# acgtun/hsearch

Measured on AMD Instinct MI355X. Metric: motif queries/sec (LSH probe + verify, index resident in HBM), higher is better.
Workload: dtype f64

## Files before the change

### hsearch_amd/capi.py

```python
import ctypes as C
import os

import numpy as np

_HERE = os.path.dirname(os.path.abspath(__file__))

HS_OK, HS_ERR_INVALID, HS_ERR_NO_DEVICE, HS_ERR_HIP, HS_ERR_CAPACITY, HS_ERR_STATE, \
    HS_ERR_KEY_COLLISION, HS_ERR_NOMEM, HS_ERR_IO, HS_ERR_PEER = range(10)
_STATUS = ["HS_OK", "HS_ERR_INVALID", "HS_ERR_NO_DEVICE", "HS_ERR_HIP", "HS_ERR_CAPACITY",
           "HS_ERR_STATE", "HS_ERR_KEY_COLLISION", "HS_ERR_NOMEM", "HS_ERR_IO", "HS_ERR_PEER"]

_ALPHABET = "ARNDCQEGHILKMFPSTWYV"

EXPORTS = ["hs_create", "hs_destroy", "hs_last_error", "hs_get_profile", "hs_get_params", "hs_version",
           "hs_set_verify_mode", "hs_set_hash_mode", "hs_set_option", "hs_set_bucket_partition", "hs_set_multiprobe", "hs_probe_buckets", "hs_wait_event", "hs_set_planes", "hs_self_join", "hs_self_join_range", "hs_clustering",
           "hs_clustering_begin", "hs_clustering_table_edges", "hs_clustering_table_apply",
           "hs_clustering_end",
           "hs_embed_codes", "hs_hash_codes", "hs_hash_points", "hs_key_string", "hs_key_fingerprint",
           "hs_key_strings_equal", "hs_index_build", "hs_index_build_subset", "hs_index_build_windows", "hs_index_shard_begin", "hs_index_shard_hash_dev", "hs_index_shard_group_dev",
           "hs_index_shard_tuples_dev", "hs_index_shard_finish_dev", "hs_index_shard_end", "hs_index_save", "hs_index_load", "hs_index_file_check", "hs_klsh_draw_planes", "hs_klsh_codes",
           "hs_index_info_get", "hs_query", "hs_query_dev", "hs_query_codes", "hs_query_codes_dev", "hs_bruteforce",
           "hs_bruteforce_topk", "hs_merge_first_table_dev", "hs_query_radii", "hs_query_radii_dev",
           "hs_bruteforce_radii", "hs_annotate", "hs_annotate_dev", "hs_merge_best", "hs_components", "hs_components_dev",
           "hs_components_range", "hs_components_range_dev", "hs_components_merge", "hs_degrees", "hs_degrees_dev",
           "hs_degrees_range", "hs_degrees_range_dev", "hs_dbscan", "hs_dbscan_dev", "hs_dbscan_edges",
           "hs_cluster_profile", "hs_cluster_profile_dev", "hs_cluster_radii", "hs_cluster_radii_dev",
           "hs_cluster_summary_codes", "hs_msf", "hs_msf_dev", "hs_msf_edges", "hs_msf_cut", "hs_core_distance",
           "hs_core_distance_dev", "hs_density_tree", "hs_density_tree_dev", "hs_density_tree_edges",
           "hs_density_tree_cut", "hs_query_topk", "hs_query_topk_dev", "hs_self_knn", "hs_self_knn_range",
           "hs_self_knn_dev", "hs_self_knn_range_dev", "hs_topk_merge", "hs_seq_match", "hs_seq_match_dev",
           "hs_window_id_start", "hs_seq_match_hits", "hs_seq_match_merge", "hs_join6_tables", "hs_join6_thresholds",
           "hs_join6_selftest", "hs_index_append", "hs_index_append_dev", "hs_index_append_windows",
           "hs_index_table_append"]

TOPK_MAX = 64
NO_ID = 0xffffffff
NOISE = 0xffffffff


class HsError(RuntimeError):
    def __init__(self, status, message):
        self.status = status
        name = _STATUS[status] if 0 <= status < len(_STATUS) else str(status)
        super().__init__("%s: %s" % (name, message))


class _Params(C.Structure):
    _fields_ = [("k", C.c_uint32), ("K", C.c_uint32), ("L", C.c_uint32), ("W", C.c_double),
                ("device", C.c_int32), ("alphabet", C.c_uint32)]


class _Profile(C.Structure):
    _fields_ = [("ms_hash", C.c_double), ("ms_sort", C.c_double), ("ms_gather", C.c_double),
                ("ms_probe", C.c_double), ("ms_verify", C.c_double), ("ms_finalize", C.c_double),
                ("ms_total", C.c_double), ("candidates", C.c_uint64), ("provisional", C.c_uint64),
                ("hits", C.c_uint64), ("verify_launches", C.c_uint64), ("join_batches", C.c_uint64),
                ("ms_join", C.c_double), ("join_items", C.c_uint64), ("join_pairs", C.c_uint64),
                ("join_pairs_issued", C.c_uint64), ("join_i8_batches", C.c_uint64),
                ("hash_values", C.c_uint64), ("hash_flagged", C.c_uint64),
                ("join_row_bytes", C.c_uint32), ("join_wide", C.c_uint32), ("join_items_resident", C.c_uint64),
                ("join_async_retries", C.c_uint64), ("queries_recognised", C.c_uint64),
                ("join_f6_batches", C.c_uint64), ("append_rebuilds", C.c_uint64),
                ("append_new_buckets", C.c_uint64)]


class _IndexInfo(C.Structure):
    _fields_ = [("n", C.c_uint64), ("device_bytes", C.c_uint64), ("n_buckets", C.c_uint64 * 32),
                ("max_bucket", C.c_uint64 * 32), ("key_seed", C.c_uint32)]


class _DbscanCounts(C.Structure):
    _fields_ = [("n_clusters", C.c_uint64), ("n_core", C.c_uint64), ("n_border", C.c_uint64),
                ("n_noise", C.c_uint64), ("n_edges", C.c_uint64)]


class _MsfInfo(C.Structure):
    _fields_ = [("n_tree_edges", C.c_uint64), ("n_components", C.c_uint64), ("n_graph_edges", C.c_uint64),
                ("rounds", C.c_uint32), ("resident", C.c_uint32)]


class _DensityInfo(C.Structure):
    _fields_ = [("n_tree_edges", C.c_uint64), ("n_clusters", C.c_uint64), ("n_core", C.c_uint64),
                ("n_graph_edges", C.c_uint64), ("rounds", C.c_uint32), ("resident", C.c_uint32),
                ("self_joins", C.c_uint32)]


profile_fields = [f[0] for f in _Profile._fields_]

_libs = {}


def lib_path(hooks=False):
    if hooks:
        return os.path.join(_HERE, "libhsearch_amd_hooks.so")
    return os.environ.get("HSEARCH_AMD_LIB") or os.path.join(_HERE, "libhsearch_amd.so")


def load(hooks=False):
    if hooks not in _libs:
        try:
            import torch
        except Exception:
            pass
        path = lib_path(hooks)
        if not os.path.exists(path):
            raise ImportError("%s is missing: run `python -c 'import __graft_entry__ as g; "
                              "g.build()'` (or make -C hsearch_amd/csrc)" % path)
        lib = C.CDLL(path)
        lib.hs_version.restype = C.c_char_p
        lib.hs_last_error.restype = C.c_char_p
        lib.hs_last_error.argtypes = [C.c_void_p]
        lib.hs_destroy.restype = None
        lib.hs_destroy.argtypes = [C.c_void_p]
        lib.hs_key_string.restype = C.c_uint32
        lib.hs_key_fingerprint.restype = C.c_uint64
        lib.hs_key_strings_equal.restype = C.c_int
        if hasattr(lib, "hs_query_radii"):
            for fn in (lib.hs_query_radii, lib.hs_query_radii_dev):
                fn.restype = C.c_int
                fn.argtypes = [C.c_void_p, C.c_void_p, C.c_void_p, C.c_uint64, C.c_void_p, C.c_void_p, C.c_void_p,
                               C.c_void_p, C.c_void_p, C.c_uint64, C.POINTER(C.c_uint64), C.c_void_p]
            lib.hs_bruteforce_radii.restype = C.c_int
            lib.hs_bruteforce_radii.argtypes = [C.c_void_p, C.c_void_p, C.c_uint64, C.c_void_p, C.c_void_p,
                                                C.c_void_p, C.c_void_p, C.c_uint64, C.POINTER(C.c_uint64)]
        if hasattr(lib, "hs_annotate"):
            for fn in (lib.hs_annotate, lib.hs_annotate_dev):
                fn.restype = C.c_int
                fn.argtypes = [C.c_void_p, C.c_void_p, C.c_void_p, C.c_uint64, C.c_double, C.c_void_p, C.c_void_p,
                               C.c_void_p, C.c_void_p, C.c_void_p, C.c_uint64, C.POINTER(C.c_uint64)]
            lib.hs_merge_best.restype = C.c_int
            lib.hs_merge_best.argtypes = [C.c_void_p, C.c_void_p, C.c_void_p, C.c_void_p, C.c_uint64, C.c_void_p,
                                          C.c_void_p, C.c_void_p, C.c_void_p, C.c_uint64, C.POINTER(C.c_uint64)]
        if hasattr(lib, "hs_components"):
            for fn in (lib.hs_components, lib.hs_components_dev):
                fn.restype = C.c_int
                fn.argtypes = [C.c_void_p, C.c_double, C.c_int, C.c_void_p, C.POINTER(C.c_uint64),
                               C.POINTER(C.c_uint64)]
            for fn in (lib.hs_components_range, lib.hs_components_range_dev):
                fn.restype = C.c_int
                fn.argtypes = [C.c_void_p, C.c_uint64, C.c_uint64, C.c_double, C.c_int, C.c_void_p,
                               C.POINTER(C.c_uint64), C.POINTER(C.c_uint64)]
            lib.hs_components_merge.restype = C.c_int
            lib.hs_components_merge.argtypes = [C.c_void_p, C.c_uint64, C.c_uint64, C.c_void_p, C.POINTER(C.c_uint64)]
        if hasattr(lib, "hs_dbscan"):
            for fn in (lib.hs_degrees, lib.hs_degrees_dev):
                fn.restype = C.c_int
                fn.argtypes = [C.c_void_p, C.c_double, C.c_int, C.c_void_p, C.POINTER(C.c_uint64)]
            for fn in (lib.hs_degrees_range, lib.hs_degrees_range_dev):
                fn.restype = C.c_int
                fn.argtypes = [C.c_void_p, C.c_uint64, C.c_uint64, C.c_double, C.c_int, C.c_void_p,
                               C.POINTER(C.c_uint64)]
            for fn in (lib.hs_dbscan, lib.hs_dbscan_dev):
                fn.restype = C.c_int
                fn.argtypes = [C.c_void_p, C.c_double, C.c_int, C.c_uint32, C.c_void_p, C.c_void_p,
                               C.POINTER(_DbscanCounts)]
            lib.hs_dbscan_edges.restype = C.c_int
            lib.hs_dbscan_edges.argtypes = [C.c_void_p, C.c_void_p, C.c_uint64, C.c_uint64, C.c_uint32, C.c_void_p,
                                            C.c_void_p, C.POINTER(_DbscanCounts)]
        if hasattr(lib, "hs_cluster_profile"):
            for fn in (lib.hs_cluster_profile, lib.hs_cluster_profile_dev):
                fn.restype = C.c_int
                fn.argtypes = [C.c_void_p, C.c_void_p, C.c_uint32, C.c_void_p, C.c_void_p, C.c_void_p, C.c_void_p,
                               C.c_uint64, C.POINTER(C.c_uint64)]
            for fn in (lib.hs_cluster_radii, lib.hs_cluster_radii_dev):
                fn.restype = C.c_int
                fn.argtypes = [C.c_void_p, C.c_void_p, C.c_uint32, C.c_void_p, C.c_uint64, C.c_void_p, C.c_void_p,
                               C.c_void_p]
            lib.hs_cluster_summary_codes.restype = C.c_int
            lib.hs_cluster_summary_codes.argtypes = [C.c_void_p, C.c_uint64, C.c_uint32, C.c_void_p, C.c_uint32,
                                                     C.c_void_p, C.c_uint32, C.c_void_p, C.c_uint64, C.c_void_p,
                                                     C.c_void_p, C.c_void_p, C.c_void_p, C.c_void_p, C.c_void_p,
                                                     C.c_void_p, C.c_uint64, C.POINTER(C.c_uint64)]
        if hasattr(lib, "hs_msf"):
            for fn in (lib.hs_msf, lib.hs_msf_dev):
                fn.restype = C.c_int
                fn.argtypes = [C.c_void_p, C.c_double, C.c_int, C.c_void_p, C.c_void_p, C.c_void_p, C.c_uint64,
                               C.c_void_p, C.POINTER(_MsfInfo)]
            lib.hs_msf_edges.restype = C.c_int
            lib.hs_msf_edges.argtypes = [C.c_void_p, C.c_void_p, C.c_void_p, C.c_uint64, C.c_uint64, C.c_void_p,
                                         C.c_void_p, C.c_void_p, C.c_uint64, C.c_void_p, C.POINTER(_MsfInfo)]
            lib.hs_msf_cut.restype = C.c_int
            lib.hs_msf_cut.argtypes = [C.c_void_p, C.c_void_p, C.c_void_p, C.c_uint64, C.c_uint64, C.c_double,
                                       C.c_void_p, C.POINTER(C.c_uint64)]
        if hasattr(lib, "hs_density_tree"):
            for fn in (lib.hs_core_distance, lib.hs_core_distance_dev):
# ... 279 lines not shown
    assert ei.ndim == 1 and ei.shape == ej.shape == dist.shape
    n = int(n)
    room = n if cap is None else int(cap)
    lo = np.empty(room, dtype=np.uint32)
    hi = np.empty(room, dtype=np.uint32)
    od = np.empty(room, dtype=np.float64)
    label = np.empty(n, dtype=np.uint32) if want_label else None
    info = _MsfInfo()
    st = load().hs_msf_edges(_vp(ei), _vp(ej), _vp(dist), len(ei), n, _vp(lo), _vp(hi), _vp(od), room,
                             _vp(label) if want_label else None, C.byref(info))
    if st != HS_OK:
        e = HsError(st, "hs_msf_edges")
        e.needed = int(info.n_tree_edges)
        raise e
    return _msf_dict(info, lo, hi, od, label)


def msf_cut(tree, r, n=None, out=None):
    lo = np.ascontiguousarray(tree["lo"], dtype=np.uint32)
    hi = np.ascontiguousarray(tree["hi"], dtype=np.uint32)
    dist = np.ascontiguousarray(tree["dist"], dtype=np.float64)
    assert lo.ndim == 1 and lo.shape == hi.shape == dist.shape
    n = len(tree["label"]) if n is None else int(n)
    if out is None:
        out = np.empty(n, dtype=np.uint32)
    assert out.dtype == np.uint32 and out.shape == (n,) and out.flags["C_CONTIGUOUS"]
    nc = C.c_uint64(0)
    st = load().hs_msf_cut(_vp(lo), _vp(hi), _vp(dist), len(lo), n, float(r), _vp(out), C.byref(nc))
    if st != HS_OK:
        raise HsError(st, "hs_msf_cut")
    return dict(label=out, n_components=int(nc.value))


def _density_dict(info, lo, hi, w, label, core):
    m = int(info.n_tree_edges)
    res = dict(lo=lo[:m], hi=hi[:m], w=w[:m], **{f[0]: int(getattr(info, f[0])) for f in _DensityInfo._fields_})
    if label is not None:
        res["label"] = label
    if core is not None:
        res["core"] = core
    return res


def density_tree_edges(ei, ej, dist, n, min_pts, want_label=True, cap=None):
    ei = np.ascontiguousarray(ei, dtype=np.uint32)
    ej = np.ascontiguousarray(ej, dtype=np.uint32)
    dist = np.ascontiguousarray(dist, dtype=np.float64)
    assert ei.ndim == 1 and ei.shape == ej.shape == dist.shape
    n = int(n)
    room = n if cap is None else int(cap)
    lo = np.empty(room, dtype=np.uint32)
    hi = np.empty(room, dtype=np.uint32)
    w = np.empty(room, dtype=np.float64)
    label = np.empty(n, dtype=np.uint32) if want_label else None
    core = np.empty(n, dtype=np.float64)
    info = _DensityInfo()
    st = load().hs_density_tree_edges(_vp(ei), _vp(ej), _vp(dist), len(ei), n, int(min_pts), _vp(lo), _vp(hi), _vp(w),
                                      room, _vp(label) if want_label else None, _vp(core), C.byref(info))
    if st != HS_OK:
        e = HsError(st, "hs_density_tree_edges")
        e.needed = int(info.n_tree_edges)
        raise e
    return _density_dict(info, lo, hi, w, label, core)


def density_tree_cut(tree, r, n=None, out=None):
    lo = np.ascontiguousarray(tree["lo"], dtype=np.uint32)
    hi = np.ascontiguousarray(tree["hi"], dtype=np.uint32)
    w = np.ascontiguousarray(tree["w"], dtype=np.float64)
    core = np.ascontiguousarray(tree["core"], dtype=np.float64)
    assert lo.ndim == 1 and lo.shape == hi.shape == w.shape and core.ndim == 1
    n = len(core) if n is None else int(n)
    assert len(core) == n
    if out is None:
        out = np.empty(n, dtype=np.uint32)
    assert out.dtype == np.uint32 and out.shape == (n,) and out.flags["C_CONTIGUOUS"]
    nc = C.c_uint64(0)
    st = load().hs_density_tree_cut(_vp(lo), _vp(hi), _vp(w), len(lo), _vp(core), n, float(r), _vp(out), C.byref(nc))
    if st != HS_OK:
        raise HsError(st, "hs_density_tree_cut")
    return dict(label=out, n_clusters=int(nc.value))


def cluster_summary_codes(codes, label, min_size=1, coords=None, centers=None, want_counts=False, want_radii=True,
                          cap=None):
    codes = np.ascontiguousarray(codes, dtype=np.uint8)
    label = np.ascontiguousarray(label, dtype=np.uint32)
    assert codes.ndim == 2 and label.shape == (codes.shape[0],)
    n, k = codes.shape
    alpha = 20
    if coords is not None:
        coords = np.ascontiguousarray(coords, dtype=np.float64)
        assert coords.ndim == 2 and coords.shape[1] == 8
        alpha = coords.shape[0]
    room = n // max(1, int(min_size)) if cap is None else int(cap)
    if centers is not None:
        centers = np.ascontiguousarray(centers, dtype=np.float64)
        assert centers.ndim == 2 and centers.shape[1] == 8 * k
    ol = np.empty(room, dtype=np.uint32)
    osz = np.empty(room, dtype=np.uint32)
    cen = np.empty((room, 8 * k), dtype=np.float64)
    cnt = np.empty((room, k, alpha), dtype=np.uint32) if want_counts else None
    mx = np.empty(room, dtype=np.float64) if want_radii else None
    rad = np.empty(room, dtype=np.float64) if want_radii else None
    med = np.empty(room, dtype=np.uint32) if want_radii else None
    n_out = C.c_uint64(0)
    opt = lambda a: None if a is None else _vp(a)
    st = load().hs_cluster_summary_codes(_vp(codes), n, k, opt(coords), alpha if coords is not None else 0, _vp(label),
                                         int(min_size), opt(centers), 0 if centers is None else centers.shape[0],
                                         _vp(ol), _vp(osz), opt(cnt), _vp(cen), opt(mx), opt(rad), opt(med), room,
                                         C.byref(n_out))
    if st != HS_OK:
        e = HsError(st, "hs_cluster_summary_codes")
        e.needed = int(n_out.value)
        raise e
    m = int(n_out.value)
    res = dict(label=ol[:m], size=osz[:m], centroid=cen[:m])
    if want_counts:
        res["counts"] = cnt[:m]
    if want_radii:
        res.update(max_d2=mx[:m], radius=rad[:m], medoid=med[:m])
    return res


def join6_tables(coords):
    coords = np.ascontiguousarray(coords, dtype=np.float64)
    A = coords.shape[0]
    s = C.c_double(0.0)
    codes = np.zeros((32, 4), dtype=np.uint8)
    e, r = np.zeros(32), np.zeros(32)
    pair = np.zeros((1024, 2), dtype=np.uint32)
    lib = load()
    st = lib.hs_join6_tables(_vp(coords), C.c_uint32(A), C.byref(s), _vp(codes), _vp(e), _vp(r), _vp(pair))
    if st:
        raise HsError(st, "hs_join6_tables")
    return dict(s=s.value, codes=codes[:A], e=e[:A], r=r[:A], pair=pair)


def join6_thresholds(coords, kmers, r2):
    coords = np.ascontiguousarray(coords, dtype=np.float64)
    kmers = np.ascontiguousarray(kmers, dtype=np.uint8)
    n, k = kmers.shape
    r2 = np.ascontiguousarray(np.broadcast_to(np.asarray(r2, dtype=np.float64), (n,)))
    rho64, c64 = np.zeros(n, dtype=np.int64), np.zeros(n, dtype=np.int64)
    rho0 = C.c_int64(0)
    rec = np.zeros((n, 4), dtype=np.uint32)
    st = load().hs_join6_thresholds(_vp(coords), C.c_uint32(coords.shape[0]), _vp(kmers), C.c_uint64(n), C.c_uint32(k),
                                    _vp(r2), _vp(rho64), _vp(c64), C.byref(rho0), _vp(rec))
    if st:
        raise HsError(st, "hs_join6_thresholds")
    return dict(rho64=rho64, c64=c64, rho0_64=rho0.value, rec=rec)


def join6_selftest(device=0, variant=0):
    n = C.c_uint64(0)
    bad = (C.c_uint32 * 4)()
    st = load().hs_join6_selftest(C.c_int(device), C.c_int(variant), C.byref(n), bad)
    if st:
        raise HsError(st, "hs_join6_selftest")
    return int(n.value), tuple(int(x) for x in bad)


def index_file_check(path):
    err = C.create_string_buffer(512)
    st = load().hs_index_file_check(str(path).encode(), err, C.c_uint32(len(err)))
    if st != HS_OK:
        raise HsError(st, err.value.decode())


def index_table_append(ids, dir_key, dir_start, dir_tuple, block_ints, seed=0, out=None):
    ids = np.ascontiguousarray(ids, dtype=np.uint32)
    dir_key = np.ascontiguousarray(dir_key, dtype=np.uint64)
    dir_start = np.ascontiguousarray(dir_start, dtype=np.uint32)
    dir_tuple = np.ascontiguousarray(dir_tuple, dtype=np.int32)
    block_ints = np.ascontiguousarray(block_ints, dtype=np.int32)
    n, nb, m = len(ids), len(dir_key), block_ints.shape[0]
    K = block_ints.shape[1] if block_ints.ndim == 2 else dir_tuple.shape[1]
    assert len(dir_start) == nb + 1 and dir_tuple.size == nb * K and block_ints.size == m * K
    lib = load()
    nb_out, collided = C.c_uint64(0), C.c_uint32(0)

    def call(o_ids, o_key, o_start, o_tuple, cap):
        return lib.hs_index_table_append(_vp(ids), _vp(dir_key), _vp(dir_start), _vp(dir_tuple), C.c_uint64(n),
                                         C.c_uint64(nb), _vp(block_ints), C.c_uint64(m), C.c_uint32(K), C.c_uint32(seed),
                                         o_ids, o_key, o_start, o_tuple, C.c_uint64(cap), C.byref(nb_out),
                                         C.byref(collided))
    if out is None:
        st = call(None, None, None, None, 0)
        if st == HS_OK and collided.value:
            return None
        if st not in (HS_OK, HS_ERR_CAPACITY):
            raise HsError(st, "hs_index_table_append")
        cap = int(nb_out.value)
        out = (np.empty(n + m, dtype=np.uint32), np.empty(cap, dtype=np.uint64), np.empty(cap + 1, dtype=np.uint32),
               np.empty((cap, K), dtype=np.int32))
    o_ids, o_key, o_start, o_tuple = out
    assert len(o_ids) >= n + m and len(o_start) >= len(o_key) + 1 and o_tuple.size >= len(o_key) * K
    st = call(_vp(o_ids), _vp(o_key), _vp(o_start), _vp(o_tuple), len(o_key))
    if st != HS_OK:
        raise HsError(st, "hs_index_table_append")
    if collided.value:
        return None
    nbo = int(nb_out.value)
    return o_ids[:n + m], o_key[:nbo], o_start[:nbo + 1], o_tuple.reshape(-1, K)[:nbo]


KLSH_NONE = 0xffffffffffffffff
_REDUCED_CLASS = {c: k for k, grp in enumerate(["AST", "RKEDQ", "NH", "C", "G", "IVLM", "FYW", "P"])
                  for c in grp}


def klsh_draw_planes(feat=512, bits=16, sigma=0.2):
    w = np.empty((bits, feat)); b = np.empty(bits); t = np.empty(bits)
    st = load().hs_klsh_draw_planes(C.c_uint32(feat), C.c_uint32(bits), C.c_double(sigma), _vp(w),
                                    _vp(b), _vp(t))
    if st != HS_OK:
        raise HsError(st, "hs_klsh_draw_planes")
    return w, b, t


def klsh_codes(classes, seq_start, w, b, t, device=0):
    classes = np.ascontiguousarray(classes, dtype=np.uint8)
    seq_start = np.ascontiguousarray(seq_start, dtype=np.uint64)
    w = np.ascontiguousarray(w, dtype=np.float64); b = np.ascontiguousarray(b, dtype=np.float64)
    t = np.ascontiguousarray(t, dtype=np.float64)
    n_seq = len(seq_start) - 1
    codes = np.empty(n_seq, dtype=np.uint64); unc = np.empty(n_seq, dtype=np.uint64)
    err = C.create_string_buffer(256)
    st = load().hs_klsh_codes(C.c_int(device), _vp(classes), C.c_uint64(len(classes)), _vp(seq_start),
                              C.c_uint64(n_seq), _vp(w), _vp(b), _vp(t), C.c_uint32(w.shape[0]),
                              _vp(codes), _vp(unc), err, C.c_uint32(256))
    if st != HS_OK:
        raise HsError(st, err.value.decode())
    return codes, unc


class Engine:

    def __init__(self, k, K, L, W, a, b, device=0, coords=None, hooks=False, options=None):
        self._lib = load(hooks)
        self.k, self.K, self.L, self.W = int(k), int(K), int(L), float(W)
        self.d = 8 * self.k
        self.T = 0
        a = np.ascontiguousarray(a, dtype=np.float64)
        b = np.ascontiguousarray(b, dtype=np.float64)
        assert a.shape == (self.L, self.K, self.d), a.shape
        assert b.shape == (self.L, self.K), b.shape
        cptr = None
        if coords is not None:
            coords = np.ascontiguousarray(coords, dtype=np.float64)
            assert coords.ndim == 2 and coords.shape[1] == 8 and 1 <= coords.shape[0] <= 32
            cptr = _vp(coords)
        params = _Params(self.k, self.K, self.L, self.W, int(device),
                         0 if coords is None else coords.shape[0])
        self._h = C.c_void_p()
        st = self._lib.hs_create(C.byref(params), _vp(a), _vp(b), cptr, C.byref(self._h))
        if st != HS_OK:
            msg = self._lib.hs_last_error(self._h).decode() if self._h else ""
            if self._h:
                self._lib.hs_destroy(self._h)
                self._h = C.c_void_p()
            raise HsError(st, msg or "hs_create failed (is a gfx950 GPU visible?)")
        for name, value in (options or {}).items():
            self.set_option(name, value)

    def _check(self, st):
        if st != HS_OK:
            raise HsError(st, self._lib.hs_last_error(self._h).decode())

    def set_verify_mode(self, mode):
        self._check(self._lib.hs_set_verify_mode(self._h, {"auto": 0, "stream": 1, "join": 2, "join16": 3}[mode]))

    def set_hash_mode(self, mode, eps_scale=1.0):
        self._check(self._lib.hs_set_hash_mode(self._h, {"auto": 0, "exact": 1, "mfma": 2}[mode],
                                               C.c_double(eps_scale)))

    OPTIONS = {"query_batch": 1, "seg_mode": 2, "join_resident": 3, "recognise_kmers": 4, "build_grouping": 5,
               "wide_rows": 6, "refine8": 7, "self_codes": 8, "sort_hits": 10, "sync_items": 11,
               "join_min_q": 12, "join_min_m": 13, "sort_from_bit": 14, "build_serial": 15,
               "join_xcd_run": 16, "probe_records": 17, "join_chunk": 18, "summary_chunk": 19, "summary_rows": 20,
               "msf_edge_budget": 21, "join_f6": 22}

    def set_option(self, name, value):
        self._check(self._lib.hs_set_option(self._h, C.c_int(self.OPTIONS[name]), C.c_int64(int(value))))

    def set_bucket_partition(self, part, n_parts):
        self._check(self._lib.hs_set_bucket_partition(self._h, C.c_uint32(part), C.c_uint32(n_parts)))

    def set_multiprobe(self, T):
        self._check(self._lib.hs_set_multiprobe(self._h, C.c_uint32(int(T))))
        self.T = int(T)

    def probe_buckets(self, centers):
        centers = np.ascontiguousarray(centers, dtype=np.float64)
        n = centers.shape[0]
        assert centers.shape == (n, self.d)
        P = self.T + 1
        buckets = np.empty((n, self.L, P, self.K), dtype=np.int32)
        valid = np.empty((n, self.L, P), dtype=np.uint8)
        self._check(self._lib.hs_probe_buckets(self._h, _vp(centers), C.c_uint64(n), _vp(buckets), _vp(valid)))
        return buckets, valid

    def wait_event(self, event_handle):
        self._check(self._lib.hs_wait_event(self._h, C.c_void_p(event_handle)))

    def set_planes(self, a, b):
# ... 736 lines not shown
```

### hsearch_amd/csrc/hs_capi.hip

```cpp
#include <math.h>
#include <random>
#include <string.h>

#include <algorithm>
#include <chrono>
#include <string>
#include <vector>

#include "../../include/hs_tables.h"
#include "hs_internal.h"
#include "hs_table_append.h"

namespace {

struct DevBuf {
  void* p = nullptr;
  size_t cap = 0;
  hipError_t reserve(size_t bytes) {
    if (bytes <= cap) return hipSuccess;
    if (p) (void)hipFree(p);
    p = nullptr;
    cap = 0;
    hipError_t e = hipMalloc(&p, bytes);
    if (e == hipSuccess) cap = bytes;
// ... 2296 lines not shown
      if (ids[i] >= n) return say(HS_ERR_IO, "id out of range" + where);
      if (seen[ids[i]]) return say(HS_ERR_IO, "id listed twice" + where);
      seen[ids[i]] = 1;
    }
    if ((nb ? start[0] : 0u) != 0u || start[nb] != n) return say(HS_ERR_IO, "bucket boundaries do not span 0..n" + where);
    for (size_t b = 0; b < nb; ++b) {
      if (!(start[b] < start[b + 1]) || start[b + 1] > n) return say(HS_ERR_IO, "bucket boundaries not ascending" + where);
      if (b + 1 < nb && !(key[b] < key[b + 1])) return say(HS_ERR_IO, "fingerprints not ascending" + where);
      if (hs_key_of(tup + b * K, (int)K, hd.key_seed) != key[b])
        return say(HS_ERR_IO, "a bucket's tuple does not have its fingerprint" + where);
      for (uint32_t i = start[b] + 1; i < start[b + 1]; ++i)
        if (!(ids[i - 1] < ids[i])) return say(HS_ERR_IO, "ids not ascending inside a bucket" + where);
    }
  }
  char extra;
  if (ph.bytes != hd.payload_bytes || ph.h != hd.payload_hash || fread(&extra, 1, 1, f) != 0)
    return say(HS_ERR_IO, "payload hash or length does not match the header");
  return HS_OK;
}

hs_status hs_index_info_get(const hs_handle* h, hs_index_info* out) {
  if (!h || !out) return HS_ERR_INVALID;
  if (!h->built) return HS_ERR_STATE;
  *out = h->info;
  return HS_OK;
}

struct BatchOut {
  uint32_t *q = nullptr, *id = nullptr, *table = nullptr;
  double* dist = nullptr;
  uint64_t room = 0;
  bool ordered = false;
};

static const hs_status HS_SPLIT_BATCH = (hs_status)1000;
static const hs_status HS_SYNC_ITEMS = (hs_status)1001;
static bool want_wide(const hs_handle* h, double R) {
  if (h->wide8) return true;
  if (!h->wide8_ok || h->p.k > 25 || h->knobs.no_wide_by_radius) return false;
  if (h->knobs.force_wide) return true;
  const double k = (double)h->p.k, sd = sqrt(k * h->pair4_var);
  return R * R > k * h->pair4_mean - 3.0 * sd;
}

static hs_status ensure_rec8w(hs_handle* h) {
  if (h->wide8 || h->rec8w_ready) return HS_OK;
  const size_t n = h->n;
  const int L = (int)h->p.L;
  HS_HIP(h, h->t_rec8w.reserve(((size_t)L * n + HS_JM_WAVE) * 16));
  for (int l = 0; l < L; ++l)
    HS_HIP(h, hs_launch_gather_rec8(h->packed_all.as<uint4>(), h->tabs.t[l].ids, (uint32_t)n, (int)h->p.k, 1,
                                    h->jtab8.p, h->jtab8.as<char>() + 1536, h->jtab8.as<float>() + 128,
                                    nullptr, h->t_rec8w.as<uint4>() + (size_t)l * n, nullptr, h->stream));
  h->rec8w_ready = true;
  return HS_OK;
}

static bool ensure_rec6(hs_handle* h) {
  if (h->rec6_state) return h->rec6_state > 0;
  const size_t n = h->n;
  const int L = (int)h->p.L;
  if (h->t_rec6.reserve(((size_t)L * n + HS_JM_WAVE) * 16) != hipSuccess) {
    (void)hipGetLastError();
    h->rec6_state = -1;
    return false;
  }
  for (int l = 0; l < L; ++l)
    if (hs_launch_gather_rec6(h->packed_all.as<uint4>(), h->tabs.t[l].ids, (uint32_t)n, (int)h->p.k, h->jtab6.p,
                              h->t_rec6.as<uint4>() + (size_t)l * n, h->stream) != hipSuccess) {
      (void)hipGetLastError();
      h->rec6_state = -1;
      return false;
    }
  h->rec6_state = 1;
  return true;
}

static bool self_codes_ok(const hs_handle* h, double R) {
  const bool wide = want_wide(h, R);
  const double r2 = R * R, s = wide ? h->join8_scale_w : h->join8_scale, k = (double)h->p.k;
  if (!h->join8_tables_ok || h->p.k > 50 || h->verify_mode == 1 || h->verify_mode == 3 || !(r2 < 30000.0))
    return false;
  if (h->join_min_q > 1 || h->join_min_m > 1 || h->knobs.no_self_codes) return false;
  return s > 0.0 && 0.5 * s * s * r2 + (wide ? 508.0 : 254.0) * k + 3.0 < 127.0 * 127.0 * 13.0;
}

struct BatchPlan {
  bool can16 = false;
  bool use_join = false;
  bool use_i8 = false;
  int wide = 0;
  bool refine = false;
  bool self_codes = false;
  bool ext_codes = false;
  bool seg_sparse = false;
  bool parted = false;
  bool all_joined = false;
  bool no_slices = false;
  bool use_r = false;
  bool f6 = false;
  uint32_t jm = HS_JM_BLOCK;
  bool async_items = false;
  uint32_t item_cap = 0;
  bool order_here = false;
  int xcd_run = -1;
  bool resident_stale = false;
};

static BatchPlan plan_batch(const hs_handle* h, const QueryCall& c, uint32_t nq, bool allow_async, bool ordered_out) {
  BatchPlan p;
  const BatchHistory& m = h->hist;
  const int k = (int)h->p.k;
  const double r2 = c.R * c.R;
  p.can16 = h->join_tables_ok && k <= 25;
  const bool can8 = h->join8_tables_ok && k <= 50 && h->verify_mode != 3;
  p.use_join = h->verify_mode != 1 && r2 < 30000.0 && (p.can16 || can8);
  p.use_i8 = p.use_join && can8;
  p.wide = (p.use_i8 && want_wide(h, c.R)) ? 1 : 0;
  p.refine = p.use_i8 && !p.wide && !h->knobs.no_refine8;
  const bool codes_ok = p.use_i8 && self_codes_ok(h, c.R);
  p.self_codes = codes_ok && c.self_first != HS_NO_SELF;
  p.ext_codes = codes_ok && c.codes;
  p.parted = p.use_join && h->bucket_parts > 1 && c.self_first == HS_NO_SELF;
  p.seg_sparse = p.parted || (h->knobs.seg_mode ? h->knobs.seg_mode == 1 : (uint64_t)h->nb_total > 2ull * nq * h->p.L);
  p.all_joined = h->join_min_q == 1 && h->join_min_m == 1;
  p.no_slices = p.use_join && p.all_joined && !p.parted;
  p.jm = p.use_i8 ? hs_join8_members_per_item(k, p.wide) : HS_JM_BLOCK;
  p.resident_stale = p.use_join && m.resident_nq && (nq > 2 * m.resident_nq || 2 * nq < m.resident_nq);
  const double share = p.resident_stale ? -1.0 : m.resident_share;
  p.use_r = p.use_i8 && !p.wide && k <= 25 && h->alphabet <= HS_JR_MAX_ALPHABET && !h->knobs.no_join_r &&
            (h->knobs.force_join_r || share < 0.0 || share >= 0.5 || m.resident_age >= 64);
  p.f6 = (p.self_codes || p.ext_codes) && !p.wide && k >= 21 && k <= 25 && h->alphabet <= 32 && h->PW == 1 &&
         h->join6_tables_ok && !h->knobs.no_join_f6 && h->rec6_state >= 0;
  p.async_items = allow_async && p.use_i8 && p.all_joined && m.item_cap_hint && !h->knobs.sync_items;
  p.item_cap = p.async_items ? m.item_cap_hint : 0;
  p.order_here = ordered_out && !h->knobs.sort_hits && !(m.order_failed && !c.radii && m.order_failed_R == c.R);
  p.xcd_run = h->knobs.join_xcd_run;
  return p;
}

struct Batch {
  uint32_t nq = 0, q_base = 0, nql = 0;
  uint32_t nqs = 0;
  double r2 = 0.0;
  const double* centers = nullptr;
  uint64_t* d_cand = nullptr;
  const uint8_t* qcodes = nullptr;
  const uint32_t* owned = nullptr;
  uint32_t n_owned = 0;
  uint32_t n_items = 0, n_slices = 1;
  const double* radii = nullptr;
};

static hipError_t launch_qrows(hs_handle* h, const BatchPlan& p, const Batch& b, hipStream_t s) {
  const int k = (int)h->p.k;
  uint32_t* const d_unsafe = h->counters.as<uint32_t>() + 8;
  if (p.f6) {
    hipError_t e = hs_launch_qprep6_codes(b.qcodes, b.nq, k, b.r2, h->jtab6.p, h->c16.as<char>() + (size_t)b.nq * 128,
                                          s, b.radii);
    if (e != hipSuccess || !p.use_r) return e;
  }
  if (p.self_codes || p.ext_codes)
    return hs_launch_qprep8_codes(b.qcodes, b.nq, k, p.wide, b.r2, h->coords.as<double>(), h->jtab8.p,
                                  h->jtab8.as<char>() + 1024, h->jtab8.as<char>() + 1536, h->jtab8.as<float>() + 128,
                                  h->c16.p, nullptr, s, b.radii);
  if (p.use_i8)
    return hs_launch_qprep8(b.centers, b.nq, k, p.wide, b.r2, h->jtab8.as<float>() + 128, h->c16.p, d_unsafe,
                            p.refine ? h->c8b.p : nullptr, s, b.radii);
  return hs_launch_qprep(b.centers, b.nq, k, b.r2, h->c16.p, d_unsafe, s, b.radii);
}

static char* c6t_of(hs_handle* h, const Batch& b) { return h->c16s.as<char>() + ((size_t)b.nql + 64) * 128; }

static hipError_t gather_qrows(hs_handle* h, const BatchPlan& p, const Batch& b) {
  if (p.f6) {
    hipError_t e = hs_launch_gather_c8t(h->c16.as<char>() + (size_t)b.nq * 128, h->sorted_ql.as<uint32_t>(),
                                        h->seg_qoff.as<uint32_t>(), h->seg_of.as<uint32_t>(), b.nqs, (int)h->p.L,
                                        (int)h->p.k, 0, c6t_of(h, b), h->stream, hs_join6_row_pieces());
    if (e != hipSuccess || !p.use_r) return e;
  }
  if (p.use_i8)
    return hs_launch_gather_c8t(h->c16.p, h->sorted_ql.as<uint32_t>(), h->seg_qoff.as<uint32_t>(),
                                h->seg_of.as<uint32_t>(), b.nqs, (int)h->p.L, (int)h->p.k, p.wide, h->c16s.p, h->stream);
  return hs_launch_gather_c16(h->c16.p, h->sorted_ql.as<uint32_t>(), b.nqs, (int)h->p.L, h->c16s.p, h->stream);
}

static hipError_t launch_probe(hs_handle* h, const QueryCall& c, const BatchPlan& p, const Batch& b) {
  uint32_t* const qbucket = p.use_join ? h->seg_keys.as<uint32_t>() : nullptr;
  uint32_t* const bucket_count = p.use_join && !p.seg_sparse ? h->bucket_work.as<uint32_t>() : nullptr;
  uint32_t* const qrank = bucket_count ? qbucket + ((size_t)b.nql + 1) : nullptr;
  unsigned long long* const d_cand_total = reinterpret_cast<unsigned long long*>(h->counters.as<uint32_t>() + 2);
  uint32_t* const nslices = (p.use_join && p.no_slices) ? nullptr : h->nslices.as<uint32_t>();
  if (p.self_codes)
    return hs_launch_self_probe(h->tabs, c.self_first + b.q_base, b.nq, (int)h->p.L, h->qstart.as<uint32_t>(),
                                h->qcount.as<uint32_t>(), nslices, b.d_cand, d_cand_total,
                                h->dir_base.as<uint32_t>(), h->nb_total, bucket_count, qbucket, qrank, h->stream);
  return hs_launch_probe(probe_tabs(h, c, b.q_base, b.owned, b.n_owned), h->qints.as<int32_t>(), b.nq, (int)h->p.K,
                         (int)h->p.L, h->key_seed, h->qstart.as<uint32_t>(), h->qcount.as<uint32_t>(),
                         nslices, b.d_cand, d_cand_total, h->probe_slow.as<uint32_t>(),
                         h->dir_base.as<uint32_t>(), h->nb_total, bucket_count, qbucket, qrank, h->stream);
}

static hs_status cut_plan_items(hs_handle* h, const BatchPlan& p, const Batch& b) {
  unsigned long long* const d_jstats = reinterpret_cast<unsigned long long*>(h->counters.as<uint32_t>() + 10);
  return cut_items(h, b.nqs, p.jm, d_jstats, p.use_r ? HS_JR_MAXQ : 0u, b.nql, !p.no_slices);
}

static hipError_t slice_offsets(hs_handle* h, const BatchPlan& p, const Batch& b) {
  if (p.use_join && p.no_slices) return hipSuccess;
  if (p.use_join && p.all_joined) return hipMemsetAsync(h->slice_off.p, 0, ((size_t)b.nql + 1) * 4, h->stream);
  return hs_exclusive_scan_u32(h->temp.p, h->temp.cap, h->nslices.as<uint32_t>(), h->slice_off.as<uint32_t>(),
                               (size_t)b.nql + 1, h->stream);
}

static hs_status prepare_queries(hs_handle* h, const QueryCall& c, const BatchPlan& p, Batch& b) {
  const int k = (int)h->p.k;
  if (p.wide) HS_CHECK(ensure_rec8w(h));
  if (p.self_codes) b.qcodes = h->codes.as<uint8_t>() + ((uint64_t)c.self_first + b.q_base) * k;
  if (c.codes) {
    HS_HIP(h, h->qcodes_buf.reserve(std::max<size_t>(16, (size_t)b.nq * k)));
    HS_HIP(h, hs_launch_check_codes(c.codes, (uint64_t)b.nq * k, h->alphabet, h->qcodes_buf.as<uint8_t>(),
                                    h->counters.as<uint32_t>() + HS_CNT_BAD_QUERY_CODE, h->stream));
    if (p.ext_codes) {
      b.qcodes = h->qcodes_buf.as<uint8_t>();
    } else {
      HS_HIP(h, h->qembed.reserve(std::max<size_t>(16, (size_t)b.nq * h->d * 8)));
      HS_HIP(h, hs_launch_embed(h->qcodes_buf.as<uint8_t>(), b.nq, k, h->coords.as<double>(),
                                h->qembed.as<double>(), h->stream));
      b.centers = h->qembed.as<double>();
    }
  }
  if (p.use_join) {
    HS_HIP(h, h->c16.reserve((size_t)b.nq * 208 * 2));
    if (p.refine && !b.qcodes) HS_HIP(h, h->c8b.reserve((size_t)b.nq * hs_join8_row_bytes(k, p.wide)));
    HS_HIP(h, hipEventRecord(h->evx[EV_FORK], h->stream));
    HS_HIP(h, hipStreamWaitEvent(h->stream2, h->evx[EV_FORK], 0));
    HS_HIP(h, launch_qrows(h, p, b, h->stream2));
    HS_HIP(h, hipEventRecord(h->evx[EV_JOIN], h->stream2));
  }
  return HS_OK;
}

static hs_status hash_and_probe(hs_handle* h, const QueryCall& c, const BatchPlan& p, Batch& b) {
  const size_t n1 = (size_t)b.nql + 1;
  HS_HIP(h, h->qints.reserve((size_t)b.nq * h->LK * 4));
  HS_HIP(h, h->qstart.reserve(((size_t)b.nql + HS_QRANGE_PAD) * 4));
  HS_HIP(h, h->qcount.reserve(((size_t)b.nql + HS_QRANGE_PAD) * 4));
  for (DevBuf* d : {&h->nslices, &h->probe_slow, &h->slice_off}) HS_HIP(h, d->reserve(n1 * 4));
  HS_HIP(h, h->temp.reserve(hs_scan_u32_temp(n1) + 256));
  if (c.pre_ints)
    HS_HIP(h, hipMemcpyAsync(h->qints.p, c.pre_ints, (size_t)b.nq * h->LK * 4, hipMemcpyDeviceToDevice, h->stream));
  else if (p.ext_codes)
    HS_CHECK(hash_dispatch(h, b.qcodes, nullptr, b.nq, -1, h->qints.as<int32_t>(), h->LK, HS_PROJ_SET_BATCH, h->stream));
  else if (!p.self_codes)
    HS_CHECK(hash_dispatch(h, nullptr, b.centers, b.nq, -1, h->qints.as<int32_t>(), h->LK, HS_PROJ_SET_BATCH, h->stream));
  HS_HIP(h, hipEventRecord(h->ev[1], h->stream));
  if (p.use_join) {
    HS_HIP(h, h->seg_keys.reserve(n1 * 8));
    HS_HIP(h, h->bucket_work.reserve(4 * (p.seg_sparse ? n1 : (size_t)h->nb_total + 2) * 4));
  }
  if (p.parted) {
    HS_HIP(h, h->part_work.reserve(5 * n1 * 4));
    uint32_t* const pw = h->part_work.as<uint32_t>();
    HS_HIP(h, hs_launch_part_owned(probe_tabs(h, c, b.q_base), h->qints.as<int32_t>(), b.nq, (int)h->p.K,
                                   (int)h->p.L, h->nb_total, pw, h->qstart.as<uint32_t>(), h->qcount.as<uint32_t>(),
                                   h->nslices.as<uint32_t>(), b.d_cand, h->seg_keys.as<uint32_t>(), h->stream));
    HS_HIP(h, hs_exclusive_scan_u32(h->temp.p, h->temp.cap, pw, pw + n1, n1, h->stream));
    HS_HIP(h, hs_launch_flagged_list(pw, pw + n1, b.nql, pw + 4 * n1, h->stream));
    HS_HIP(h, hipMemcpyAsync(&b.n_owned, pw + n1 + b.nql, 4, hipMemcpyDeviceToHost, h->stream));
    HS_HIP(h, hipStreamSynchronize(h->stream));
    b.owned = pw + 4 * n1;
  }
  HS_HIP(h, launch_probe(h, c, p, b));
  return HS_OK;
}

static hs_status group_segments(hs_handle* h, const BatchPlan& p, Batch& b) {
  if (!p.use_join) return HS_OK;
  const size_t n1 = (size_t)b.nql + 1;
  HS_HIP(h, h->c16s.reserve(((size_t)b.nql + 64) * 208 * 2));
  for (DevBuf* d : {&h->seg_keys, &h->seg_keys_sorted, &h->seg_key}) HS_HIP(h, d->reserve(n1 * 8));
  for (DevBuf* d : {&h->seg_vals, &h->sorted_ql, &h->seg_cnt, &h->seg_qoff, &h->seg_items, &h->item_off, &h->seg_of})
    HS_HIP(h, d->reserve(n1 * 4));
  HS_HIP(h, h->seg_n.reserve(64));
  HS_HIP(h, h->temp.reserve(std::max(hs_scan_u32_temp(n1), hs_scan_u32_temp((size_t)h->nb_total + 2)) + 256));
  HS_HIP(h, hipStreamWaitEvent(h->stream, h->evx[EV_JOIN], 0));
  const int L = (int)h->p.L, seg_shift = seg_shift_of(h);
  if (p.seg_sparse) {
    HS_HIP(h, h->temp.reserve(std::max(hs_sort_pairs_u32_u32_temp(b.nql), hs_scan_u32_temp(n1)) + 256));
    const uint32_t* keys_in = h->seg_keys.as<uint32_t>();
    const uint32_t* probes_in = nullptr;
    if (p.parted) {
      uint32_t* const pw = h->part_work.as<uint32_t>();
      uint32_t n_found = 0;
      if (b.n_owned) {
        HS_HIP(h, hs_launch_found_probes(h->seg_keys.as<uint32_t>(), b.n_owned, h->nb_total, h->temp.p, h->temp.cap,
                                         pw, pw + n1, pw + 2 * n1, pw + 3 * n1, h->stream, b.owned));
        HS_HIP(h, hipMemcpyAsync(&n_found, pw + n1 + b.n_owned, 4, hipMemcpyDeviceToHost, h->stream));
      }
      HS_HIP(h, hipStreamSynchronize(h->stream));
      if (n_found) {
        b.nqs = n_found;
        keys_in = pw + 2 * n1;
        probes_in = pw + 3 * n1;
      }
    }
    HS_HIP(h, hs_launch_seg_group_sparse(h->tabs, h->dir_base.as<uint32_t>(), L, seg_shift, h->nb_total, h->temp.p,
                                         h->temp.cap, keys_in, h->seg_keys.as<uint32_t>() + n1,
                                         h->seg_vals.as<uint32_t>(), h->bucket_work.as<uint32_t>(), b.nqs,
                                         h->sorted_ql.as<uint32_t>(), h->seg_key.as<uint64_t>(),
                                         h->seg_cnt.as<uint32_t>(), h->seg_n.as<uint32_t>(), h->seg_of.as<uint32_t>(),
                                         h->stream, probes_in));
  } else {
    HS_HIP(h, hs_launch_seg_group(h->tabs, h->dir_base.as<uint32_t>(), L, seg_shift, h->nb_total,
                                  h->bucket_work.as<uint32_t>(),
                                  h->bucket_work.as<uint32_t>() + (((size_t)h->nb_total + 3) & ~(size_t)1),
                                  h->temp.p, h->temp.cap, h->seg_keys.as<uint32_t>(), h->seg_keys.as<uint32_t>() + n1,
                                  b.nql, h->sorted_ql.as<uint32_t>(), h->seg_key.as<uint64_t>(),
                                  h->seg_cnt.as<uint32_t>(), h->seg_n.as<uint32_t>(), h->seg_of.as<uint32_t>(),
                                  h->stream));
  }
  HS_HIP(h, hs_exclusive_scan_u32(h->temp.p, h->temp.cap, h->seg_cnt.as<uint32_t>(), h->seg_qoff.as<uint32_t>(),
                                  (size_t)b.nqs + 1, h->stream));
  HS_CHECK(cut_plan_items(h, p, b));
  HS_HIP(h, gather_qrows(h, p, b));
  return HS_OK;
}

static hs_status demote(hs_handle* h, const QueryCall& c, BatchPlan& p, Batch& b, uint32_t unsafe) {
  if (p.self_codes || p.ext_codes) return fail(h, HS_ERR_STATE, "queries from codes: a query row marked unsafe");
  uint32_t* const d_cnt = h->counters.as<uint32_t>();
  if (p.use_i8) {
    p.use_i8 = p.refine = false;
    if (p.can16) {
      HS_HIP(h, hipMemsetAsync(d_cnt + 8, 0, 4, h->stream));
      HS_HIP(h, launch_qrows(h, p, b, h->stream));
      HS_HIP(h, gather_qrows(h, p, b));
      HS_HIP(h, hipMemcpyAsync(&unsafe, d_cnt + 8, 4, hipMemcpyDeviceToHost, h->stream));
      if (p.jm != HS_JM_BLOCK) {
        p.jm = HS_JM_BLOCK;
        p.use_r = false;
        HS_HIP(h, hipMemsetAsync(d_cnt + 10, 0, 16, h->stream));
        HS_CHECK(cut_plan_items(h, p, b));
        HS_HIP(h, hipMemcpyAsync(&b.n_items, h->item_off.as<uint32_t>() + b.nqs, 4, hipMemcpyDeviceToHost,
                                 h->stream));
      }
      HS_HIP(h, hipStreamSynchronize(h->stream));
    }
  }
  if (unsafe) {
    p.use_join = false;
    b.n_items = 0;
    b.owned = nullptr;
    b.n_owned = 0;
    HS_HIP(h, hipMemsetAsync(d_cnt + 2, 0, 8, h->stream));
    HS_HIP(h, hipMemsetAsync(h->probe_slow.p, 0, 4, h->stream));
    HS_HIP(h, launch_probe(h, c, p, b));
    HS_HIP(h, slice_offsets(h, p, b));
    b.n_slices = 1;
  }
  return HS_OK;
}

static hs_status read_items(hs_handle* h, const QueryCall& c, BatchPlan& p, Batch& b) {
  HS_HIP(h, slice_offsets(h, p, b));
  uint32_t unsafe = 0;
  if (p.async_items) {
    b.n_items = p.item_cap;
    b.n_slices = 0;
  } else {
    if (p.use_join) {
      HS_HIP(h, hipMemcpyAsync(&unsafe, h->counters.as<uint32_t>() + 8, 4, hipMemcpyDeviceToHost, h->stream));
      HS_HIP(h, hipMemcpyAsync(&b.n_items, h->item_off.as<uint32_t>() + b.nqs, 4, hipMemcpyDeviceToHost, h->stream));
    }
    HS_HIP(h, hipMemcpyAsync(&b.n_slices, h->slice_off.as<uint32_t>() + b.nql, 4, hipMemcpyDeviceToHost, h->stream));
    HS_HIP(h, hipStreamSynchronize(h->stream));
  }
  if (unsafe) HS_CHECK(demote(h, c, p, b, unsafe));
  if (b.n_items) {
    HS_HIP(h, h->item_desc.reserve((size_t)b.n_items * 32));
    HS_HIP(h, hs_launch_item_desc(h->tabs, h->seg_key.as<uint64_t>(), h->seg_cnt.as<uint32_t>(),
                                  h->seg_qoff.as<uint32_t>(), h->item_off.as<uint32_t>(), b.nqs,
                                  h->sorted_ql.as<uint32_t>(), h->qcount.as<uint32_t>(), b.n_items, p.jm,
                                  seg_shift_of(h), h->seg_vals.as<uint32_t>(), h->PW,
                                  p.async_items ? h->item_off.as<uint32_t>() + b.nqs : nullptr,
                                  h->seg_res.as<uint64_t>(), h->seg_n.as<uint32_t>() + 2,
                                  h->counters.as<uint32_t>() + HS_CNT_SPLIT, h->item_desc.as<uint4>(), h->stream));
  }
  if (b.n_slices) {
    HS_HIP(h, h->tq.reserve((size_t)b.nq * h->p.k * HS_TROW * 4));
    if (!b.n_items)
      HS_HIP(h, hs_launch_qtables(b.centers, b.nq, (int)h->p.k, h->coords.as<double>(), h->alphabet,
                                  h->tq.as<float>(), h->stream));
  }
  return HS_OK;
}

static hs_status launch_filters(hs_handle* h, const BatchPlan& p, const Batch& b, uint32_t prov_cap, bool again) {
  const int k = (int)h->p.k, L = (int)h->p.L;
  const float r2_hi = filter_bound(b.r2);
  uint32_t* const d_cnt = h->counters.as<uint32_t>();
  const int n_blocks = h->n_cu * 8, join_blocks = h->n_cu * h->join_blocks_per_cu;
  const bool side = b.n_items && b.n_slices;
  auto verify = [&](hipStream_t s) {
    return hs_launch_verify(h->tabs, h->qstart.as<uint32_t>(), h->qcount.as<uint32_t>(), h->slice_off.as<uint32_t>(),
                            b.nql, h->tq.as<float>(), k, L, r2_hi, d_cnt, prov_cap, h->prov.as<uint2>(), n_blocks, s,
                            b.radii);
  };
  if (side) {
    HS_HIP(h, hipEventRecord(h->evx[EV_FORK], h->stream));
    HS_HIP(h, hipStreamWaitEvent(h->stream2, h->evx[EV_FORK], 0));
    if (!again)
      HS_HIP(h, hs_launch_qtables(b.centers, b.nq, k, h->coords.as<double>(), h->alphabet, h->tq.as<float>(),
                                  h->stream2));
    HS_HIP(h, verify(h->stream2));
    HS_HIP(h, hipEventRecord(h->evx[EV_JOIN], h->stream2));
  }
  HS_HIP(h, hipEventRecord(h->ev[11], h->stream));
  if (b.n_items && p.use_i8) {
    const uint32_t* const d_split = h->seg_n.as<uint32_t>() + 2;
    const uint4* const rec8 = (p.wide && !h->wide8) ? h->t_rec8w.as<uint4>() : h->t_rec8.as<uint4>();
    const void* const rows = p.wide ? (const void*)(h->jtab8.as<char>() + 1536) : (const void*)h->jtab8.p;
    const uint64_t tile_bytes = (uint64_t)b.nqs * (uint64_t)hs_join8_row_bytes(k, p.wide);
    const uint32_t xcd_run = p.xcd_run >= 0 ? (uint32_t)p.xcd_run : (tile_bytes > (64ull << 20) ? 128u : 0u);
    const uint32_t* const d_n_items =
        p.use_r ? d_split : (p.async_items ? h->item_off.as<uint32_t>() + b.nqs : nullptr);
    if (p.f6)
      HS_HIP(h, hs_launch_join6x(h->item_desc.as<uint4>(), b.n_items, h->tabs.t[0].packed, h->t_rec6.as<uint4>(),
                                 c6t_of(h, b), h->jtab6.p, d_cnt, prov_cap, h->prov.as<uint2>(), d_cnt + 32,
                                 join_blocks, d_n_items,
                                 hs_join8_chunk_items(b.n_items, join_blocks, h->hist.pairs_per_item,
                                                      h->knobs.join_chunk),
                                 xcd_run, h->stream));
// ... 2165 lines not shown
```

### hsearch_amd/csrc/hs_internal.h

```cpp
#ifndef HS_INTERNAL_H
#define HS_INTERNAL_H

#include <hip/hip_runtime.h>
#include <stdint.h>
#include <string.h>

#include "../../include/hsearch.h"

#define HS_MAX_L 32
#define HS_MAX_K 32
#define HS_ALPHABET_PAD 32
#define HS_TROW 32
#define HS_PROV_INDIRECT 0x80000000u
#define HS_SLICE 4096u
#define HS_KEY_CHARS (11 * HS_MAX_K + 1)

#include "hs_key.h"

#define HS_CNT_SURVIVOR_OVERFLOW 21
#define HS_CNT_BAD_QUERY_CODE 22
#define HS_CNT_PROJ 48
#define HS_CNT_SPLIT 50
#define HS_CNT_WORDS 64
#ifdef __HIPCC__
// ... 310 lines not shown
                              const uint64_t* d_id_start, uint64_t n_seq, uint64_t n, uint64_t* d_out, hipStream_t s);
hipError_t hs_launch_sm_key(const uint64_t* d_key, const uint64_t* d_val, const uint32_t* d_q, const uint32_t* d_id,
                            const double* d_dist, uint32_t n_hits, const uint32_t* d_q_group, const uint32_t* d_q_off,
                            const uint64_t* d_id_start, uint64_t n_seq, int ws, int wd, uint64_t max_qoff,
                            uint64_t* d_out_key, uint32_t* d_out_idx, hipStream_t s);
hipError_t hs_launch_sm_iota(uint32_t n, uint32_t* d_idx, hipStream_t s);
hipError_t hs_launch_sm_head(const uint64_t* d_skey, uint32_t n, uint32_t* d_head, hipStream_t s);
size_t hs_sm_part_bytes(uint32_t n);
hipError_t hs_launch_sm_reduce(const uint64_t* d_skey, const uint32_t* d_sidx, const uint32_t* d_excl,
                               const uint32_t* d_head, uint32_t n, const uint64_t* d_key, const uint64_t* d_val,
                               const uint32_t* d_q, const uint32_t* d_id, const double* d_dist,
                               const uint64_t* d_id_start, int ws, int wd, const void* d_src_rows, uint64_t src_cap,
                               void* d_dst_rows, uint64_t dst_cap, uint64_t dst_row0, uint32_t n_rows, void* d_part,
                               hipStream_t s);
hipError_t hs_launch_sm_decode(const void* d_rows, uint64_t cap, uint32_t n, int ws, int wd, uint64_t max_qoff,
                               uint32_t* d_group, uint32_t* d_seq, int32_t* d_diag, uint32_t* d_count,
                               double* d_best_dist, uint32_t* d_best_q, uint32_t* d_best_id, uint32_t* d_lo,
                               uint32_t* d_hi, uint32_t* d_flag, hipStream_t s);
hipError_t hs_launch_cc_begin(uint32_t* d_parent, uint32_t n, uint64_t* d_counts, hipStream_t s);
hipError_t hs_launch_cc_union(const uint64_t* d_key, uint32_t n_hits, uint32_t self_first, uint32_t* d_parent,
                              uint32_t n, uint64_t* d_counts, hipStream_t s);
hipError_t hs_launch_cc_flatten(uint32_t* d_parent, uint32_t n, uint32_t* d_label, uint64_t* d_counts, hipStream_t s);
hipError_t hs_launch_db_begin(uint32_t* d_deg, uint32_t* d_parent, uint32_t* d_anchor, uint32_t n, uint64_t* d_counts,
                              hipStream_t s);
hipError_t hs_launch_db_degree(const uint64_t* d_key, uint32_t n_hits, uint32_t self_first, uint32_t* d_deg, uint32_t n,
                               uint64_t* d_counts, hipStream_t s);
hipError_t hs_launch_db_unite(const uint64_t* d_key, uint32_t n_hits, uint32_t self_first, const uint32_t* d_deg,
                              uint32_t min_pts, uint32_t* d_parent, uint32_t* d_anchor, uint32_t n, hipStream_t s);
hipError_t hs_launch_db_finish(uint32_t* d_parent, const uint32_t* d_deg, const uint32_t* d_anchor, uint32_t min_pts,
                               uint32_t n, uint32_t* d_label, uint64_t* d_counts, hipStream_t s);
#define HS_MSF_MAX_ROUNDS 34u
hipError_t hs_launch_msf_begin(uint32_t* d_comp, uint32_t* d_parent, uint64_t* d_best_d, uint64_t* d_best_pair,
                               uint32_t n, uint64_t* d_counts, hipStream_t s);
hipError_t hs_launch_msf_min_d_hits(const uint64_t* d_key, const uint64_t* d_val, uint32_t n_hits, uint32_t self_first,
                                    const uint32_t* d_comp, uint64_t* d_best_d, uint32_t n, uint64_t* d_counts,
                                    void* d_kept, uint64_t kept_cap, hipStream_t s);
hipError_t hs_launch_msf_min_pair_hits(const uint64_t* d_key, const uint64_t* d_val, uint32_t n_hits,
                                       uint32_t self_first, const uint32_t* d_comp, const uint64_t* d_best_d,
                                       uint64_t* d_best_pair, uint32_t n, hipStream_t s);
hipError_t hs_launch_msf_min_d_kept(const void* d_kept, uint64_t n_kept, const uint32_t* d_comp, uint64_t* d_best_d,
                                    uint32_t n, uint64_t* d_counts, hipStream_t s);
hipError_t hs_launch_msf_min_pair_kept(const void* d_kept, uint64_t n_kept, const uint32_t* d_comp,
                                       const uint64_t* d_best_d, uint64_t* d_best_pair, uint32_t n, hipStream_t s);
hipError_t hs_launch_msf_select(uint32_t* d_comp, uint32_t* d_parent, uint64_t* d_best_d, uint64_t* d_best_pair,
                                uint32_t n, uint64_t* d_out_pair, uint64_t* d_out_d, uint64_t* d_counts,
                                hipStream_t s);
hipError_t hs_launch_msf_finish(const uint32_t* d_comp, uint32_t n, uint32_t* d_label, uint64_t* d_counts,
                                hipStream_t s);
hipError_t hs_launch_msf_unpack(const uint64_t* d_pair, const uint64_t* d_d, uint32_t m, uint32_t* d_lo, uint32_t* d_hi,
                                double* d_dist, hipStream_t s);
hipError_t hs_launch_dt_begin(uint64_t* d_core, uint64_t* d_thr, uint64_t* d_next, uint32_t* d_cnt, uint32_t n,
                              uint32_t min_pts, hipStream_t s);
hipError_t hs_launch_dt_pairs(const uint64_t* d_key, const uint64_t* d_val, uint32_t n_hits, uint32_t self_first,
                              uint32_t n, uint64_t* d_counts, void* d_kept, uint64_t kept_cap, hipStream_t s);
hipError_t hs_launch_dt_round(const uint64_t* d_key, const uint64_t* d_val, uint32_t n_hits, uint32_t self_first,
                              uint32_t n, uint32_t first, uint32_t count, uint32_t min_pts, uint64_t* d_core,
                              uint64_t* d_thr, uint64_t* d_next, uint32_t* d_cnt, uint64_t* d_counts, hipStream_t s);
hipError_t hs_launch_dt_core_finish(uint64_t* d_core, uint32_t n, uint64_t* d_counts, hipStream_t s);
hipError_t hs_launch_dt_min_d_hits(const uint64_t* d_key, const uint64_t* d_val, uint32_t n_hits, uint32_t self_first,
                                   const uint64_t* d_core, const uint32_t* d_comp, uint64_t* d_best_d, uint32_t n,
                                   uint64_t* d_counts, hipStream_t s);
hipError_t hs_launch_dt_min_pair_hits(const uint64_t* d_key, const uint64_t* d_val, uint32_t n_hits,
                                      uint32_t self_first, const uint64_t* d_core, const uint32_t* d_comp,
                                      const uint64_t* d_best_d, uint64_t* d_best_pair, uint32_t n, hipStream_t s);
hipError_t hs_launch_dt_min_d_kept(const void* d_kept, uint64_t n_kept, const uint64_t* d_core, const uint32_t* d_comp,
                                   uint64_t* d_best_d, uint32_t n, uint64_t* d_counts, hipStream_t s);
hipError_t hs_launch_dt_min_pair_kept(const void* d_kept, uint64_t n_kept, const uint64_t* d_core,
                                      const uint32_t* d_comp, const uint64_t* d_best_d, uint64_t* d_best_pair,
                                      uint32_t n, hipStream_t s);
hipError_t hs_launch_dt_finish(const uint32_t* d_comp, const uint64_t* d_core, uint32_t n, uint32_t* d_label,
                               uint64_t* d_counts, hipStream_t s);
hipError_t hs_launch_sm_group(const uint32_t* d_label, uint32_t n, uint32_t min_size, uint32_t* d_size, uint32_t* d_tmp,
                              uint32_t* d_row_of, uint32_t* d_off_of, void* d_temp, size_t temp_bytes, uint32_t* d_err,
                              hipStream_t s);
hipError_t hs_launch_sm_members(const uint32_t* d_label, uint32_t n, uint32_t min_size, const uint32_t* d_size,
                                const uint32_t* d_row_of, uint32_t* d_off_of, uint32_t* d_row_label,
                                uint32_t* d_row_off, uint32_t* d_member, hipStream_t s);
hipError_t hs_launch_sm_head(const uint32_t* d_row_label, const uint32_t* d_row_off, uint32_t n_rows,
                             uint32_t* d_out_label, uint32_t* d_out_size, hipStream_t s);
hipError_t hs_launch_sm_profile(const uint8_t* d_codes, int k, int alphabet, const uint32_t* d_label,
                                const uint32_t* d_row_of, const uint32_t* d_row_off, const uint32_t* d_member,
                                uint32_t r0, uint32_t r1, uint32_t ch, uint32_t n_kept, uint32_t* d_counts,
                                int n_cu, hipStream_t s);
hipError_t hs_launch_sm_centroid(const uint32_t* d_counts, const double* d_coords, int k, int alphabet,
                                 const uint32_t* d_row_off, uint32_t r0, uint32_t r1, double* d_centroid,
                                 hipStream_t s);
hipError_t hs_launch_sm_radii(const uint8_t* d_codes, int k, int alphabet, const double* d_coords,
                              const uint32_t* d_label, const uint32_t* d_row_of, const uint32_t* d_row_off,
                              const uint32_t* d_member, uint32_t n_rows, uint32_t n_kept, uint32_t ch,
                              const double* d_centers, uint64_t* d_d2, double* d_max_d2, double* d_radius,
                              uint32_t* d_medoid, int n_cu, hipStream_t s);
hipError_t hs_launch_bruteforce(const uint4* d_packed_all, uint32_t n, const float* d_tq,
                                uint32_t nq, int k, float r2_hi, uint32_t* d_prov_count,
                                uint32_t prov_cap, uint2* d_prov, const float* d_q_thr,
                                float* d_slice_min, int n_blocks, hipStream_t s, const double* d_radii = nullptr);
hipError_t hs_launch_jtables(const double* d_coords, int alphabet, void* d_tab16, float* d_rownorm,
                             uint32_t* d_unsafe, hipStream_t s);
hipError_t hs_launch_qprep(const double* d_centers, uint32_t nq, int k, double r2, void* d_c16,
                           uint32_t* d_unsafe, hipStream_t s, const double* d_radii = nullptr);
hipError_t hs_launch_seg_route(const uint64_t* d_seg_key, const uint32_t* d_seg_cnt,
                               const uint32_t* d_seg_qoff, const uint32_t* d_n_seg,
                               const uint32_t* d_sorted_ql, const uint32_t* d_qcount, uint32_t n_max,
                               uint32_t min_q, uint32_t min_m, uint32_t jm, int L, int shift,
                               uint32_t max_q_resident ,
                               uint32_t big_min_q, uint32_t* d_items, uint64_t* d_class,
                               unsigned long long* d_stats, uint32_t* d_nslices, const uint32_t* d_seg_of,
                               hipStream_t s);
hipError_t hs_launch_item_desc(const hs_tables_dev& tabs, const uint64_t* d_seg_key,
                               const uint32_t* d_seg_cnt,
                               const uint32_t* d_seg_qoff, const uint32_t* d_item_off, uint32_t n_max,
                               const uint32_t* d_sorted_ql, const uint32_t* d_qcount, uint32_t n_items,
                               uint32_t jm, int shift, const uint32_t* d_order, int PW,
                               const uint32_t* d_n_items ,
                               const uint64_t* d_class_pos ,
                               uint32_t* d_split ,
                               uint32_t* d_split_copy ,
                               uint4* d_desc, hipStream_t s);
hipError_t hs_launch_seg_order(const uint64_t* d_class_pos, const uint32_t* d_items, uint32_t n, uint32_t* d_order,
                               uint32_t* d_items_ordered, hipStream_t s);
#define HS_JR_MAXQ 64u
#define HS_JR_MAX_ALPHABET 24
#define HS_JM_BLOCK 512u
#define HS_JM_WAVE 128u
#ifndef HS_JQG_WAVE
#define HS_JQG_WAVE 8192u
#endif
hipError_t hs_launch_gather_c16(const void* d_c16, const uint32_t* d_sorted_ql, uint32_t nql, int L,
                                void* d_out, hipStream_t s);
hipError_t hs_launch_join(const uint4* d_desc, uint32_t n_items, const uint4* d_packed_base,
                          const uint32_t* d_sorted_ql, const void* d_c16s, const void* d_tab16,
                          const float* d_rownorm, int k, uint32_t* d_prov_count, uint32_t prov_cap,
                          uint2* d_prov, int n_blocks, hipStream_t s);
hipError_t hs_launch_jtables8(const double* d_coords, int alphabet, void* d_tab8, float* d_scale,
                              uint32_t* d_unsafe, void* d_tabR, void* d_tabW, hipStream_t s);
hipError_t hs_launch_qprep8_codes(const uint8_t* d_qcodes, uint32_t nq, int k, int wide, double r2,
                                  const double* d_coords, const void* d_tab8, const void* d_tabR,
                                  const void* d_tabW, const float* d_scale, void* d_c8, void* d_c8b,
                                  hipStream_t s, const double* d_radii = nullptr);
hipError_t hs_launch_qprep8(const double* d_centers, uint32_t nq, int k, int wide, double r2,
                            const float* d_scale, void* d_c8, uint32_t* d_unsafe, void* d_c8b,
                            hipStream_t s, const double* d_radii = nullptr);
hipError_t hs_launch_refine8(const hs_tables_dev& tabs, const uint2* d_prov, const uint32_t* d_prov_count,
                             uint32_t prov_cap, const uint32_t* d_sorted_ql, const void* d_c8,
                             const void* d_c8b, const void* d_tabR, const float* d_scale, int k, int L,
                             const uint32_t* d_qstart, const uint32_t* d_qcount,
                             uint2* d_out, uint32_t* d_out_count, hipStream_t s);
hipError_t hs_launch_refine_codes(const hs_tables_dev& tabs, const uint2* d_prov, const uint32_t* d_prov_count,
                                  uint32_t prov_cap, const uint32_t* d_sorted_ql, const uint4* d_qpacked,
                                  const double* d_coords, int alphabet, int k, int L, double r2,
                                  const double* d_radii, const uint32_t* d_qstart, const uint32_t* d_qcount,
                                  uint2* d_out, uint32_t* d_out_count, hipStream_t s);
hipError_t hs_launch_gather_c8t(const void* d_c8, const uint32_t* d_sorted_ql, const uint32_t* d_seg_qoff,
                                const uint32_t* d_seg_of, uint32_t nql, int L, int k, int wide, void* d_out,
                                hipStream_t s, int pieces = 0 );
int hs_join8_row_bytes(int k, int wide);
uint32_t hs_join8_members_per_item(int k, int wide);
uint32_t hs_join8_chunk_items(uint32_t n_items, int n_blocks, double pairs_per_item, uint32_t chunk);
size_t hs_join6_table_bytes();
size_t hs_join6_ok_offset();
int hs_join6_row_pieces();
hipError_t hs_launch_jtables6(const double* d_coords, int alphabet, void* d_tab6, hipStream_t s);
hipError_t hs_launch_gather_rec6(const uint4* d_packed_all, const uint32_t* d_ids_sorted, uint32_t n, int k,
                                 const void* d_tab6, uint4* d_out_rec, hipStream_t s);
hipError_t hs_launch_qprep6_codes(const uint8_t* d_qcodes, uint32_t nq, int k, double r2, const void* d_tab6,
                                  void* d_c6, hipStream_t s, const double* d_radii = nullptr);
hipError_t hs_launch_join6x(const uint4* d_desc, uint32_t n_items, const uint4* d_packed_base,
                            const uint4* d_rec_base, const void* d_c6t, const void* d_tab6, uint32_t* d_prov_count,
                            uint32_t prov_cap, uint2* d_prov, uint32_t* d_item_counter, int n_blocks,
                            const uint32_t* d_n_items, uint32_t G, uint32_t xcd_run, hipStream_t s);
hipError_t hs_launch_join8w(const uint4* d_desc, uint32_t n_items, const uint4* d_packed_base,
                            const uint4* d_rec_base, const void* d_c8t, const void* d_tab8, int k, int wide,
                            uint32_t* d_prov_count, uint32_t prov_cap, uint2* d_prov,
                            uint32_t* d_item_counter, int n_blocks, const uint32_t* d_n_items,
                            double pairs_per_item, uint32_t xcd_run, hipStream_t s, uint32_t chunk = 0);
hipError_t hs_launch_join8r(const uint4* d_desc, uint32_t desc_cap, const uint32_t* d_split,
                            const uint4* d_packed_base, const uint32_t* d_rho_base ,
                            const void* d_c8t,
                            const void* d_tab8, int alphabet , uint32_t* d_prov_count, uint32_t prov_cap,
                            uint2* d_prov, uint32_t* d_item_counter, int n_blocks, double pairs_per_item,
                            hipStream_t s);
hipError_t hs_launch_gather_rec8(const uint4* d_packed_all, const uint32_t* d_ids_sorted, uint32_t n,
                                 int k, int wide, const void* d_tab8, const void* d_tabW, const float* d_scale,
                                 uint4* d_out_packed, uint4* d_out_rec,
                                 uint32_t* d_out_rho ,
                                 hipStream_t s);
hipError_t hs_launch_kth_min(const float* d_slice_min, uint32_t nq, uint32_t per_q, uint32_t topk,
                             float* d_thr, hipStream_t s);
hipError_t hs_launch_topk_exact(const uint8_t* d_codes, const double* d_centers,
                                const double* d_coords, const uint2* d_prov,
                                const uint32_t* d_prov_count, uint32_t prov_cap, int k,
                                uint64_t* d_key, uint64_t* d_val, hipStream_t s);
hipError_t hs_launch_bf_finalize(const uint8_t* d_codes, const double* d_centers,
                                 const double* d_coords, const uint2* d_prov,
                                 const uint32_t* d_prov_count, uint32_t prov_cap, int k, double R,
                                 uint32_t q_base, uint32_t* d_hit_count, uint32_t hit_cap,
                                 uint64_t* d_hit_key, uint64_t* d_hit_val, hipStream_t s,
                                 const double* d_radii = nullptr );
hipError_t hs_launch_radii_max(const double* d_radii, uint64_t n, unsigned long long* d_out, hipStream_t s);

hipError_t hs_launch_append_match(const uint64_t* d_bkey, const int32_t* d_btuple, uint32_t nbB, int K,
                                  const uint64_t* d_dir_key, const int32_t* d_dir_tuple, const uint32_t* d_dir_jump,
                                  uint32_t jump_shift, uint32_t nb, uint32_t* d_pos, uint32_t* d_is_new,
                                  uint32_t* d_inc, uint32_t* d_flag, hipStream_t s);
hipError_t hs_launch_append_dir(const uint64_t* d_dir_key, const uint32_t* d_dir_start, const int32_t* d_dir_tuple,
                                uint32_t nb, const uint64_t* d_bkey, const uint32_t* d_bstart, const int32_t* d_btuple,
                                uint32_t nbB, int K, const uint32_t* d_pos, const uint32_t* d_is_new,
                                const uint32_t* d_new_scan, const uint32_t* d_inc, const uint32_t* d_inc_scan,
                                uint32_t* d_map_old, uint32_t* d_map_blk, uint32_t* d_old_cnt, uint64_t* d_out_key,
                                int32_t* d_out_tuple, uint32_t* d_out_count, hipStream_t s);
hipError_t hs_launch_append_bases(const uint32_t* d_out_start, const uint32_t* d_dir_start, const uint32_t* d_map_old,
                                  uint32_t nb, const uint32_t* d_bstart, const uint32_t* d_map_blk,
                                  const uint32_t* d_old_cnt, uint32_t nbB, uint32_t* d_base_old, uint32_t* d_base_blk,
                                  hipStream_t s);
hipError_t hs_launch_append_move(uint32_t n_src, const uint32_t* d_seg_start, uint32_t n_seg, const uint32_t* d_base,
                                 uint32_t n_dst, int PW, const uint32_t* d_src_ids, uint32_t id_add,
                                 const uint4* d_src_packed, const uint4* d_src_rec, const uint32_t* d_src_rho,
                                 uint32_t* d_dst_ids, uint4* d_dst_packed, uint4* d_dst_rec, uint32_t* d_dst_rho,
                                 hipStream_t s);

#endif
```

### hsearch_amd/csrc/hs_join6.hip

```cpp
#include <stddef.h>
#include <stdio.h>
#include <stdlib.h>
#include <string.h>

#include <algorithm>
#include <vector>

#include "hs_internal.h"
#include "hs_join6_tables.h"

namespace {

typedef int intx6 __attribute__((ext_vector_type(6)));
typedef int intx8 __attribute__((ext_vector_type(8)));
typedef float floatx4 __attribute__((ext_vector_type(4)));

constexpr uint32_t JRES = 256;
constexpr int PIECES = 7;

__device__ __forceinline__ void close_reservation(uint2* __restrict__ prov, uint32_t res_base, uint32_t res_used,
                                                  uint32_t prov_cap, int lane) {
  for (uint32_t i = res_used + (uint32_t)lane; i < JRES; i += 64u)
    if (res_base + i < prov_cap) prov[res_base + i] = make_uint2(0xffffffffu, 0u);
}

__device__ __forceinline__ uint4 uniform4(const uint4 v) {
  return make_uint4(__builtin_amdgcn_readfirstlane(v.x), __builtin_amdgcn_readfirstlane(v.y),
                    __builtin_amdgcn_readfirstlane(v.z), __builtin_amdgcn_readfirstlane(v.w));
}

template <int SCALE = 0>
__device__ __forceinline__ floatx4 tile_mfma6(const intx6 a, const intx6 b, const floatx4 c) {
  const intx8 a8 = __builtin_shufflevector(a, a, 0, 1, 2, 3, 4, 5, -1, -1);
  const intx8 b8 = __builtin_shufflevector(b, b, 0, 1, 2, 3, 4, 5, -1, -1);
  return __builtin_amdgcn_mfma_scale_f32_16x16x128_f8f6f4(a8, b8, c, 2, 2, 0, SCALE, 0, SCALE);
}

__global__ void hs_jtables6_kernel(const double* __restrict__ coords, int alphabet, hs_j6_dev* __restrict__ T) {
  if (threadIdx.x == 0 && blockIdx.x == 0) hs_j6_compute(coords, alphabet, T, nullptr, nullptr);
}

__global__ __launch_bounds__(256) void hs_gather_rec6_kernel(const uint4* __restrict__ packed_all,
                                                             const uint32_t* __restrict__ ids, uint32_t n, int k,
                                                             const hs_j6_dev* __restrict__ T,
                                                             uint4* __restrict__ out_rec) {
  __shared__ double sR[32];
  __shared__ uint32_t sBits[32];
  if (threadIdx.x < 32) {
    sR[threadIdx.x] = T->r[threadIdx.x];
    sBits[threadIdx.x] = T->bits[threadIdx.x];
  }
  __syncthreads();
  const uint32_t t = blockIdx.x * 256 + threadIdx.x;
  if (t >= n) return;
  const uint4 pk = packed_all[ids[t]];
  const uint32_t w[4] = {pk.x, pk.y, pk.z, pk.w};
  double rho = 0.0;
  uint32_t pos24 = 0;
#pragma unroll
  for (int p = 0; p < 25; ++p) {
    const int bit = 5 * p, wi = bit >> 5, sh = bit & 31;
    uint32_t c = w[wi] >> sh;
    if (sh > 27) c |= w[wi + 1] << (32 - sh);
    c &= 31u;
    if (p < k) {
      rho += sR[c];
      if (p == 24) pos24 = sBits[c];
    }
  }
  uint32_t rec[4];
  hs_j6_record(rho, k, T->rpos64, pos24, rec, nullptr);
  out_rec[t] = make_uint4(rec[0], rec[1], rec[2], rec[3]);
}

__global__ __launch_bounds__(256) void hs_qprep6_codes_kernel(const uint8_t* __restrict__ qcodes, uint32_t nq, int k,
                                                              double r2_call, const hs_j6_dev* __restrict__ T,
                                                              uint32_t* __restrict__ out,
                                                              const double* __restrict__ radii) {
  __shared__ double sR[32];
  __shared__ uint32_t sBits[32];
  if (threadIdx.x < 32) {
    sR[threadIdx.x] = T->r[threadIdx.x];
    sBits[threadIdx.x] = T->bits[threadIdx.x];
  }
  __syncthreads();
  const uint32_t q = blockIdx.x * 256 + threadIdx.x;
  if (q >= nq) return;
  const double r2 = hs_r2_of(radii, q, r2_call);
  const uint8_t* code = qcodes + (uint64_t)q * k;
  uint32_t W[4][6];
#pragma unroll
  for (int a = 0; a < 4; ++a)
#pragma unroll
    for (int i = 0; i < 6; ++i) W[a][i] = 0u;
  hs_j6_query_consts(W[3]);
  double sum_r = 0.0;
#pragma unroll
  for (int p = 0; p < 25; ++p) {
    if (p < k) {
      const uint32_t c = code[p] & 31u;
      sum_r += sR[c];
      const uint32_t b = sBits[c];
      const int qu = p >> 3, bit = 24 * (p & 7), wi = bit >> 5, sh = bit & 31;
      W[qu][wi] |= b << sh;
      if (sh > 8) W[qu][wi + 1] |= b >> (32 - sh);
    }
  }
  int64_t c64 = hs_j6_query_c64(sum_r, T->s2_half, r2, k, T->rpos64);
  c64 = c64 > HS_J6_CMAX ? HS_J6_CMAX : c64 < -HS_J6_CMAX ? -HS_J6_CMAX : c64;
  if (!(r2 == r2)) c64 = -HS_J6_CMAX;
  uint32_t* row = out + (uint64_t)q * (PIECES * 4);
#pragma unroll
  for (int a = 0; a < 4; ++a) {
#pragma unroll
    for (int i = 0; i < 4; ++i) row[4 * a + i] = W[a][i];
    row[16 + 4 * (a >> 1) + 2 * (a & 1)] = W[a][4];
    row[16 + 4 * (a >> 1) + 2 * (a & 1) + 1] = W[a][5];
  }
  row[24] = __float_as_uint((float)c64 * (1.0f / 64.0f));
  row[25] = row[26] = row[27] = 0u;
}

__device__ __forceinline__ void load_btile6(intx6 (&B)[2], float (&C)[2], const uint4* __restrict__ c6t,
                                            uint32_t row0, uint32_t nr, int lane) {
  const char* t0 = reinterpret_cast<const char*>(c6t + (uint64_t)row0 * PIECES);
  const uint32_t n = (uint32_t)lane & 15u, q = (uint32_t)lane >> 4;
#pragma unroll
  for (int c = 0; c < 2; ++c) {
    const uint32_t row = min(16u * (uint32_t)c + n, nr - 1u);
    const uint4 hi = *reinterpret_cast<const uint4*>(t0 + (q * nr + row) * 16u);
    const uint2 lo = *reinterpret_cast<const uint2*>(t0 + ((4u + (q >> 1)) * nr + row) * 16u + 8u * (q & 1u));
    C[c] = *reinterpret_cast<const float*>(t0 + (6u * nr + row) * 16u);
    B[c] = intx6{(int)hi.x, (int)hi.y, (int)hi.z, (int)hi.w, (int)lo.x, (int)lo.y};
  }
}

__device__ __forceinline__ void sign_step6(int g, const floatx4 (&acc)[4][2], int (&w)[16]) {
  auto v = [&](int i) { return __float_as_int(acc[i >> 3][(i >> 2) & 1][i & 3]); };
  if (g < 10) w[g] = max(max(v(3 * g), v(3 * g + 1)), v(3 * g + 2));
  else if (g < 13) w[g] = max(max(w[3 * (g - 10)], w[3 * (g - 10) + 1]), w[3 * (g - 10) + 2]);
  else if (g == 13) w[13] = max(max(w[9], v(30)), v(31));
  else if (g == 14) w[14] = max(max(w[10], w[11]), w[12]);
  else w[15] = max(w[13], w[14]);
  asm volatile("" : "+v"(w[g]));
}

__device__ __forceinline__ uint32_t and_tree6(const floatx4 (&acc)[4][2]) {
  uint32_t a = 0xffffffffu;
#pragma unroll
  for (int t = 0; t < 4; ++t)
#pragma unroll
    for (int c = 0; c < 2; ++c)
#pragma unroll
      for (int i = 0; i < 4; ++i) a &= __float_as_uint(acc[t][c][i]);
  return a;
}

__device__ __forceinline__ void emit_survivors6(const floatx4 (&acc)[4][2], int T0, uint32_t qc, uint32_t qoff,
                                                uint32_t q_end, uint32_t wbase, uint32_t M, uint32_t mstart,
                                                int lane, uint32_t& res_base, uint32_t& res_used,
                                                uint32_t* __restrict__ prov_count, uint32_t prov_cap,
                                                uint2* __restrict__ prov) {
  const uint32_t n = (uint32_t)lane & 15u, q = (uint32_t)lane >> 4;
#pragma unroll
  for (int t = 0; t < 4; ++t)
#pragma unroll
    for (int c = 0; c < 2; ++c) {
      const uint32_t any = __float_as_uint(acc[t][c][0]) & __float_as_uint(acc[t][c][1]) &
                           __float_as_uint(acc[t][c][2]) & __float_as_uint(acc[t][c][3]);
      if (!__ballot((int)any >= 0)) continue;
      uint32_t mask = 0;
#pragma unroll
      for (int i = 0; i < 4; ++i) mask |= (__float_as_int(acc[t][c][i]) >= 0 ? 1u : 0u) << i;
      const uint32_t col = qc + 16u * (uint32_t)c + n;
      if (!(col < q_end)) mask = 0u;
      const uint32_t ql = HS_PROV_INDIRECT | (qoff + col);
      while (__ballot(mask != 0)) {
        uint32_t idx = 0;
        bool pass = false;
        if (mask) {
          const int i = __ffs((int)mask) - 1;
          mask &= mask - 1;
          idx = wbase + (uint32_t)(16 * (T0 + t)) + 4u * q + (uint32_t)i;
          pass = idx < M;
        }
        const unsigned long long m = __ballot(pass);
        if (m) {
          const uint32_t cnt = (uint32_t)__popcll(m);
          if (res_used + cnt > JRES) {
            close_reservation(prov, res_base, res_used, prov_cap, lane);
            uint32_t base = 0;
            if (lane == 0) base = hs_reserve_survivors(prov_count, (uint32_t)JRES);
            res_base = __builtin_amdgcn_readfirstlane(base);
            res_used = 0;
          }
          if (pass) {
            const uint32_t o = res_base + res_used + (uint32_t)__popcll(m & ((1ull << lane) - 1ull));
            if (o < prov_cap) prov[o] = make_uint2(ql, mstart + idx);
          }
          res_used += cnt;
        }
      }
    }
}

__global__ __launch_bounds__(256, 2) void hs_join6x_kernel(
    const uint4* __restrict__ desc, uint32_t n_items, const uint4* __restrict__ packed_base,
    const uint4* __restrict__ rec_base, const uint4* __restrict__ c6t, const hs_j6_dev* __restrict__ T,
    uint32_t* __restrict__ prov_count, uint32_t prov_cap, uint2* __restrict__ prov,
    uint32_t* __restrict__ item_counter, uint32_t G, const uint32_t* __restrict__ n_items_dev, uint32_t xcd_run) {
  if (n_items_dev) n_items = min(n_items, __builtin_amdgcn_readfirstlane(*n_items_dev));
  constexpr int RT = 8;
  __shared__ uint2 sPair[1024];
  const int tid = threadIdx.x, lane = tid & 63;
  const int wave = __builtin_amdgcn_readfirstlane(tid >> 6);
  const int n = lane & 15, q = lane >> 4;
  for (int e = tid; e < 1024; e += 256) sPair[e] = T->pair[e];
  __syncthreads();
  const uint32_t xcd_sh = 31u - (uint32_t)__builtin_clz(xcd_run | 1u), xcd_mask = (1u << xcd_sh) - 1u;
  uint32_t victim = __builtin_amdgcn_s_getreg(6164) & 7u;
  uint32_t tried = 0;
  const uint32_t first_dynamic = gridDim.x * 4u * G;
  auto chunk_item = [&](uint32_t v) -> uint32_t {
    if (!xcd_run) return first_dynamic + v;
    for (;;) {
      const uint32_t c = ((((v >> xcd_sh) << 3) + victim) << xcd_sh) + (v & xcd_mask);
      const uint64_t it = (uint64_t)c * G;
      if (it < (uint64_t)n_items) return (uint32_t)it;
      if (++tried == 8u) return 0xf0000000u;
      victim = (victim + 1u) & 7u;
      uint32_t j = 0;
      if (lane == 0) j = atomicAdd(item_counter + 8 + victim, 1u);
      v = __builtin_amdgcn_readfirstlane(j);
    }
  };
#define HS_TAKE_CHUNK() (xcd_run ? atomicAdd(item_counter + 8 + victim, 1u) : atomicAdd(item_counter, G))
  uint32_t item = (blockIdx.x * 4u + (uint32_t)wave) * G;
  if (xcd_run) {
    uint32_t first = 0;
    if (lane == 0) first = HS_TAKE_CHUNK();
    item = chunk_item(__builtin_amdgcn_readfirstlane(first));
  }
  if (item >= n_items) return;
  uint32_t res_base = 0, res_used = JRES;
  uint32_t next_chunk_v = 0;
  if (lane == 0) next_chunk_v = HS_TAKE_CHUNK();
  uint32_t pf_item = item, pf_chunk_end = min(item + G, n_items);
#define HS_ADVANCE_PF()                                                                  \
  {                                                                                      \
    ++pf_item;                                                                           \
    if (pf_item == pf_chunk_end) {                                                       \
      pf_item = chunk_item(__builtin_amdgcn_readfirstlane(next_chunk_v));                \
      pf_chunk_end = pf_item < n_items ? min(pf_item + G, n_items) : pf_item + G;        \
      if (lane == 0 && pf_item < n_items) next_chunk_v = HS_TAKE_CHUNK();                \
    }                                                                                    \
  }
  uint4 d0 = uniform4(desc[2 * (uint64_t)item]), d1 = uniform4(desc[2 * (uint64_t)item + 1]);
  HS_ADVANCE_PF()
  uint32_t next_item = pf_item;
  uint4 nd0 = d0, nd1 = d1;
  if (next_item < n_items) {
    nd0 = uniform4(desc[2 * (uint64_t)next_item]);
    nd1 = uniform4(desc[2 * (uint64_t)next_item + 1]);
  }
  uint4 mk[RT];
  constexpr int NB = 3;
  constexpr uint32_t GQ = 32 * NB;
  intx6 Bq[NB][2];
  float Cq[NB][2];
#define HS_LOAD_MEMBERS(D0)                                                              \
  {                                                                                      \
    const int64_t off_ = (int64_t)(((uint64_t)(D0).y << 32) | (uint64_t)(D0).x);         \
    const uint4* src_ = (q == 3 ? rec_base : packed_base) + off_;                        \
    const uint32_t idx_ = (D0).w * 128u + (uint32_t)n;                                   \
    _Pragma("unroll") for (int t = 0; t < RT; ++t)                                       \
      mk[t] = src_[min(idx_ + 16 * t, (D0).z - 1)];                                      \
  }
  const uint32_t skew = ((blockIdx.x * 4u + (uint32_t)wave) * 40503u) & 0xffffu;
#define HS_N_GROUPS(D1) (((D1).z - (D1).y + GQ - 1u) / GQ)
#define HS_FIRST_Q(D1) ((D1).y + GQ * ((skew * HS_N_GROUPS(D1)) >> 16))
#define HS_LOAD_GROUP(ROW, Q0, QEND)                                                             \
  _Pragma("unroll") for (int u = 0; u < NB; ++u) {                                               \
    const uint32_t qu_ = (Q0) + 32u * u < (QEND) ? (Q0) + 32u * u : (Q0);                        \
    load_btile6(Bq[u], Cq[u], c6t, (ROW) + qu_, min(32u, (QEND) - qu_), lane);                   \
  }
  HS_LOAD_MEMBERS(d0)
  {
    const uint32_t q0 = HS_FIRST_Q(d1);
    HS_LOAD_GROUP(d1.x, q0, d1.z)
  }
  const uint32_t bs = 8u * (uint32_t)min(q, 2);
  while (true) {
    const uint32_t M = d0.z, mt = d0.w;
    const uint32_t qoff = d1.x, q_begin = d1.y, q_end = d1.z, mstart = d1.w;
    const uint32_t wbase = mt * 128u;
    const bool has_next = next_item < n_items;
    HS_ADVANCE_PF()
    uint4 nnd0 = nd0, nnd1 = nd1;
    if (pf_item < n_items) {
      nnd0 = uniform4(desc[2 * (uint64_t)pf_item]);
      nnd1 = uniform4(desc[2 * (uint64_t)pf_item + 1]);
    }
    intx6 A[RT];
#pragma unroll
    for (int t = 0; t < RT; ++t) {
      const uint4 m = mk[t];
      const uint32_t a = q == 0 ? m.x : q == 1 ? m.y : m.z, b = q == 0 ? m.y : q == 1 ? m.z : m.w;
      const uint32_t lo = __funnelshift_r(a, b, bs), hi = b >> bs;
      const uint2 e0 = sPair[lo & 1023u], e1 = sPair[(lo >> 10) & 1023u];
      const uint2 e2 = sPair[(lo >> 20) & 1023u], e3 = sPair[__funnelshift_r(lo, hi, 30) & 1023u];
      const intx6 lk = intx6{(int)e0.x, (int)(e0.y | (e1.x << 16)), (int)__funnelshift_r(e1.x, e1.y, 16),
                             (int)e2.x, (int)(e2.y | (e3.x << 16)), (int)__funnelshift_r(e3.x, e3.y, 16)};
      const intx6 own = intx6{(int)m.x, (int)m.y, (int)m.z, (int)m.w, 0, 0};
      A[t] = q == 3 ? own : lk;
    }
    HS_LOAD_MEMBERS(nd0)
    floatx4 accX[4][2], accY[4][2];
#pragma unroll
    for (int t = 0; t < 4; ++t)
#pragma unroll
      for (int c = 0; c < 2; ++c) accY[t][c] = __builtin_nondeterministic_value(accY[t][c]);
    bool y_live = false;
    uint32_t prev_qc = q_begin;
    const uint32_t n_groups = HS_N_GROUPS(d1);
    uint32_t qc0 = HS_FIRST_Q(d1);
    auto do_group = [&](uint32_t gi) {
      uint32_t nrow = qoff, nq0 = qc0 + GQ, nqend = q_end;
      if (nq0 >= q_end) nq0 = q_begin;
      if (gi + 1 == n_groups) {
        nrow = nd1.x;
        nq0 = HS_FIRST_Q(nd1);
        nqend = nd1.z;
      }
#pragma unroll
      for (int u = 0; u < NB; ++u) {
        const uint32_t qc = qc0 + 32u * (uint32_t)u;
        intx6 (&B)[2] = Bq[u];
        if (u == 0 || qc < q_end) {
          const floatx4 Cv[2] = {floatx4{Cq[u][0], Cq[u][0], Cq[u][0], Cq[u][0]},
                                 floatx4{Cq[u][1], Cq[u][1], Cq[u][1], Cq[u][1]}};
          int wY[16];
#pragma unroll
          for (int g = 0; g < 8; ++g) {
            const int t = g >> 1, c = g & 1;
            accX[t][c] = tile_mfma6(A[t], B[c], Cv[c]);
            if (y_live) {
              sign_step6(2 * g, accY, wY);
              sign_step6(2 * g + 1, accY, wY);
            }
            __builtin_amdgcn_sched_barrier(0);
          }
          const uint32_t sY = y_live ? (uint32_t)wY[15] : 0x80000000u;
          if (y_live && __ballot((int)sY >= 0))
            emit_survivors6(accY, 4, prev_qc, qoff, q_end, wbase, M, mstart, lane, res_base, res_used, prov_count,
                            prov_cap, prov);
          y_live = true;
          int wX[16];
#pragma unroll
          for (int g = 0; g < 8; ++g) {
            const int t = g >> 1, c = g & 1;
            accY[t][c] = tile_mfma6(A[4 + t], B[c], Cv[c]);
            sign_step6(2 * g, accX, wX);
            sign_step6(2 * g + 1, accX, wX);
            __builtin_amdgcn_sched_barrier(0);
          }
          const uint32_t sX = (uint32_t)wX[15];
          if (__ballot((int)sX >= 0))
            emit_survivors6(accX, 0, qc, qoff, q_end, wbase, M, mstart, lane, res_base, res_used, prov_count,
                            prov_cap, prov);
          prev_qc = qc;
        }
        const uint32_t nb = nq0 + 32u * (uint32_t)u < nqend ? nq0 + 32u * (uint32_t)u : nq0;
        load_btile6(B, Cq[u], c6t, nrow + nb, min(32u, nqend - nb), lane);
      }
      qc0 = nq0;
    };
    do_group(0);
    for (uint32_t gi = 1; gi < n_groups; ++gi) do_group(gi);
    {
      const uint32_t sY = and_tree6(accY);
      if (__ballot((int)sY >= 0))
        emit_survivors6(accY, 4, prev_qc, qoff, q_end, wbase, M, mstart, lane, res_base, res_used, prov_count,
                        prov_cap, prov);
    }
    if (!has_next) break;
    item = next_item;
    next_item = pf_item;
    d0 = nd0;
    d1 = nd1;
    nd0 = nnd0;
    nd1 = nnd1;
  }
#undef HS_ADVANCE_PF
#undef HS_TAKE_CHUNK
#undef HS_LOAD_GROUP
#undef HS_N_GROUPS
#undef HS_LOAD_MEMBERS
#undef HS_FIRST_Q
  close_reservation(prov, res_base, res_used, prov_cap, lane);
}

__device__ __forceinline__ uint32_t st_hash(uint32_t x) {
  x ^= x >> 16;
  x *= 0x7feb352du;
  x ^= x >> 15;
  x *= 0x846ca68bu;
  x ^= x >> 16;
  return x;
}
__device__ __forceinline__ uint32_t st_code(uint32_t cs, uint32_t side, uint32_t row, uint32_t k) {
  const uint32_t MAXP = 31u, MAXN = 63u;
  if (cs == 0) return MAXP;
  if (cs == 1) return side ? MAXN : MAXP;
  if (cs == 2) return side ? MAXP : ((k & 1u) ? MAXN : MAXP);
  if (cs == 3) return ((k + (side ? 0u : row)) & 1u) ? MAXN : MAXP;
  if ((cs & 1u) && k >= 117u) return 0u;
  return st_hash(cs * 0x9e3779b9u + side * 0x85ebca6bu + row * 131u + k * 2654435761u) & 63u;
}
__device__ __forceinline__ int32_t st_c64(uint32_t cs, uint32_t col) {
  const int32_t big = 1 << 23;
  if (cs == 0) return big;
  if (cs == 1) return -big;
  if (cs == 2) return big - 1;
  if (cs == 3) return -(big - 1);
  return (int32_t)(st_hash(cs * 977u + col * 0x27d4eb2fu) % (uint32_t)(2 * big + 1)) - big;
}
template <int SCALE>
__global__ __launch_bounds__(64) void hs_join6_selftest_kernel(uint32_t* __restrict__ mismatches,
                                                               uint32_t* __restrict__ first_bad) {
  const uint32_t cs = blockIdx.x, lane = threadIdx.x & 63u, n = lane & 15u, q = lane >> 4;
  uint32_t a[6] = {0, 0, 0, 0, 0, 0}, b[6] = {0, 0, 0, 0, 0, 0};
#pragma unroll
  for (int i = 0; i < 32; ++i) {
    const uint32_t ca = st_code(cs, 0u, n, 32u * q + (uint32_t)i), cb = st_code(cs, 1u, n, 32u * q + (uint32_t)i);
    const int bit = 6 * i, wi = bit >> 5, sh = bit & 31;
    a[wi] |= ca << sh;
    b[wi] |= cb << sh;
    if (sh > 26) {
      a[wi + 1] |= ca >> (32 - sh);
      b[wi + 1] |= cb >> (32 - sh);
    }
  }
  const float cf = (float)st_c64(cs, n) * (1.0f / 64.0f);
  const floatx4 d = tile_mfma6<SCALE>(intx6{(int)a[0], (int)a[1], (int)a[2], (int)a[3], (int)a[4], (int)a[5]},
                                      intx6{(int)b[0], (int)b[1], (int)b[2], (int)b[3], (int)b[4], (int)b[5]},
                                      floatx4{cf, cf, cf, cf});
#pragma unroll
  for (int i = 0; i < 4; ++i) {
    const uint32_t row = 4u * q + (uint32_t)i;
    long long ref = (long long)st_c64(cs, n);
    for (uint32_t k = 0; k < 128u; ++k)
      ref += (long long)hs_e2m3_eighths(st_code(cs, 0u, row, k)) * (long long)hs_e2m3_eighths(st_code(cs, 1u, n, k));
    const double got = (double)d[i] * 64.0;
    if (!(got == (double)ref)) {
      if (atomicAdd(mismatches, 1u) == 0u) {
        first_bad[0] = cs;
        first_bad[1] = lane * 4u + (uint32_t)i;
        first_bad[2] = __float_as_uint(d[i]);
        first_bad[3] = (uint32_t)(int32_t)ref;
      }
    }
  }
}

inline unsigned blocks_for(uint64_t n, unsigned per = 256) { return (unsigned)((n + per - 1) / per); }

}

hipError_t hs_launch_jtables6(const double* d_coords, int alphabet, void* d_tab6, hipStream_t s) {
  hs_jtables6_kernel<<<1, 64, 0, s>>>(d_coords, alphabet, (hs_j6_dev*)d_tab6);
  return hipGetLastError();
}

size_t hs_join6_table_bytes() { return sizeof(hs_j6_dev); }
size_t hs_join6_ok_offset() { return offsetof(hs_j6_dev, ok); }
int hs_join6_row_pieces() { return PIECES; }

hipError_t hs_launch_gather_rec6(const uint4* d_packed_all, const uint32_t* d_ids_sorted, uint32_t n, int k,
                                 const void* d_tab6, uint4* d_out_rec, hipStream_t s) {
  if (!n) return hipSuccess;
  hs_gather_rec6_kernel<<<blocks_for(n), 256, 0, s>>>(d_packed_all, d_ids_sorted, n, k, (const hs_j6_dev*)d_tab6,
                                                      d_out_rec);
  return hipGetLastError();
}

hipError_t hs_launch_qprep6_codes(const uint8_t* d_qcodes, uint32_t nq, int k, double r2, const void* d_tab6,
                                  void* d_c6, hipStream_t s, const double* d_radii) {
  if (!nq) return hipSuccess;
  hs_qprep6_codes_kernel<<<blocks_for(nq), 256, 0, s>>>(d_qcodes, nq, k, r2, (const hs_j6_dev*)d_tab6,
                                                        (uint32_t*)d_c6, d_radii);
  return hipGetLastError();
}

hipError_t hs_launch_join6x(const uint4* d_desc, uint32_t n_items, const uint4* d_packed_base,
                            const uint4* d_rec_base, const void* d_c6t, const void* d_tab6, uint32_t* d_prov_count,
                            uint32_t prov_cap, uint2* d_prov, uint32_t* d_item_counter, int n_blocks,
                            const uint32_t* d_n_items, uint32_t G, uint32_t xcd_run, hipStream_t s) {
  if (!n_items) return hipSuccess;
  hs_join6x_kernel<<<n_blocks, 256, 0, s>>>(d_desc, n_items, d_packed_base, d_rec_base, (const uint4*)d_c6t,
                                            (const hs_j6_dev*)d_tab6, d_prov_count, prov_cap, d_prov, d_item_counter,
                                            G, d_n_items, xcd_run);
  return hipGetLastError();
}

extern "C" {

HS_API hs_status hs_join6_tables(const double* coords, uint32_t alphabet, double* s, uint8_t* codes, double* e,
                                 double* r, uint32_t* pair) {
  if (!coords || alphabet < 1 || alphabet > 32) return HS_ERR_INVALID;
  std::vector<hs_j6_dev> T(1);
  double ee[32], ss = 0.0;
  hs_j6_compute(coords, (int)alphabet, &T[0], ee, &ss);
  if (!T[0].ok) return HS_ERR_INVALID;
  if (s) *s = ss;
  for (int a = 0; a < 32; ++a) {
    if (codes)
      for (int j = 0; j < 4; ++j) codes[a * 4 + j] = (uint8_t)((T[0].bits[a] >> (6 * j)) & 63u);
    if (e) e[a] = ee[a];
    if (r) r[a] = T[0].r[a];
  }
  if (pair) memcpy(pair, T[0].pair, sizeof(T[0].pair));
  return HS_OK;
}

HS_API hs_status hs_join6_thresholds(const double* coords, uint32_t alphabet, const uint8_t* kmers, uint64_t n,
                                     uint32_t k, const double* r2, int64_t* rho64, int64_t* c64, int64_t* rho0_64,
                                     uint32_t* rec) {
  if (!coords || alphabet < 1 || alphabet > 32 || !kmers || k < 1 || k > 25) return HS_ERR_INVALID;
  std::vector<hs_j6_dev> T(1);
  hs_j6_compute(coords, (int)alphabet, &T[0], nullptr, nullptr);
  if (!T[0].ok) return HS_ERR_INVALID;
  if (rho0_64) *rho0_64 = (int64_t)k * T[0].rpos64;
  for (uint64_t i = 0; i < n; ++i) {
    double sum = 0.0;
    uint32_t pos24 = 0;
    for (uint32_t p = 0; p < k; ++p) {
      const uint32_t c = kmers[i * k + p];
      if (c >= alphabet) return HS_ERR_INVALID;
      sum += T[0].r[c];
      if (p == 24) pos24 = T[0].bits[c];
    }
    uint32_t w[4];
    int64_t enc = 0;
    hs_j6_record(sum, (int)k, T[0].rpos64, pos24, w, &enc);
    if (rho64) rho64[i] = enc;
    if (rec) memcpy(rec + 4 * i, w, 16);
    if (c64) {
      int64_t c = hs_j6_query_c64(sum, T[0].s2_half, r2 ? r2[i] : 0.0, (int)k, T[0].rpos64);
      c64[i] = c > HS_J6_CMAX ? HS_J6_CMAX : c < -HS_J6_CMAX ? -HS_J6_CMAX : c;
    }
  }
  return HS_OK;
}

HS_API hs_status hs_join6_selftest(int device, int variant, uint64_t* mismatches, uint32_t* first_bad) {
  if (!mismatches || variant < 0 || variant > 1) return HS_ERR_INVALID;
  if (hipSetDevice(device) != hipSuccess) return HS_ERR_HIP;
  uint32_t* d = nullptr;
  if (hipMalloc(reinterpret_cast<void**>(&d), 32) != hipSuccess) return HS_ERR_HIP;
  uint32_t host[8] = {0, 0, 0, 0, 0, 0, 0, 0};
  hipError_t e = hipMemset(d, 0, 32);
  if (e == hipSuccess) {
    constexpr int CASES = 64;
    if (variant == 0) hs_join6_selftest_kernel<0><<<CASES, 64>>>(d, d + 1);
    else hs_join6_selftest_kernel<127><<<CASES, 64>>>(d, d + 1);
    e = hipGetLastError();
  }
  if (e == hipSuccess) e = hipMemcpy(host, d, 32, hipMemcpyDeviceToHost);
  (void)hipFree(d);
  if (e != hipSuccess) return HS_ERR_HIP;
  *mismatches = host[0];
  if (first_bad) memcpy(first_bad, host + 1, 16);
  return HS_OK;
}

}
```

### hsearch_amd/csrc/hs_join6_tables.h

```cpp
#pragma once
#include <math.h>
#include <stdint.h>

struct hs_j6_dev {
  uint2 pair[1024];
  double r[32];
  uint32_t bits[32];
  double s2_half;
  int32_t rpos64;
  int32_t ok;
};

#define HS_J6_NC 15
#define HS_J6_QMAX (15 * HS_J6_NC)

__host__ __device__ inline int hs_e2m3_eighths(uint32_t c) {
  const int m = (int)(c & 7u), e = (int)((c >> 3) & 3u);
  const int v = e ? (8 + m) << (e - 1) : m;
  return (c & 32u) ? -v : v;
}
__host__ __device__ inline uint32_t hs_e2m3_code(int v8) {
  const uint32_t sg = v8 < 0 ? 32u : 0u;
  const uint32_t a = (uint32_t)(v8 < 0 ? -v8 : v8);
  return sg | (a < 16u ? a : a < 32u ? (a >> 1) + 8u : (a >> 2) + 16u);
}
__host__ __device__ inline uint32_t hs_e2m3_nearest(double v) {
  const double a = fabs(v);
  uint32_t best = 0;
  double bd = a;
  for (uint32_t c = 1; c < 32u; ++c) {
    const double d = fabs(a - 0.125 * (double)hs_e2m3_eighths(c));
    if (d < bd) {
      bd = d;
      best = c;
    }
  }
  return best | ((v < 0.0 && best) ? 32u : 0u);
}

__host__ __device__ inline void hs_j6_compute(const double* coords, int alphabet, hs_j6_dev* T, double* e_out,
                                              double* s_out) {
  double mm = 0.0;
  for (int a = 0; a < alphabet && a < 32; ++a)
    for (int j = 0; j < 4; ++j) mm = fmax(mm, fabs(coords[a * 8 + j]));
  T->ok = (mm > 0.0 && mm < 1e6 && alphabet >= 1 && alphabet <= 32) ? 1 : 0;
  if (!T->ok) mm = 1.0;
  const double s = 7.5 / mm;
  int X8[32][4];
  double e[32];
  for (int a = 0; a < 32; ++a) {
    uint32_t b = 0;
    for (int j = 0; j < 4; ++j) {
      const uint32_t c = (a < alphabet && T->ok) ? hs_e2m3_nearest(s * coords[a * 8 + j]) : 0u;
      X8[a][j] = hs_e2m3_eighths(c);
      b |= c << (6 * j);
    }
    T->bits[a] = b;
    e[a] = 0.0;
    T->r[a] = 0.0;
  }
  auto E = [&](int a, int b) {
    double dot = 0.0;
    int S = 0;
    for (int j = 0; j < 4; ++j) {
      dot += coords[a * 8 + j] * coords[b * 8 + j];
      S += X8[a][j] * X8[b][j];
    }
    return s * s * dot - (double)S / 64.0;
  };
  if (T->ok) {
    for (int a = 0; a < alphabet; ++a) {
      double m = E(a, a);
      for (int b = 0; b < alphabet; ++b) m = fmax(m, E(a, b));
      e[a] = 0.5 * m;
    }
    for (int sweep = 0; sweep < 200; ++sweep) {
      bool moved = false;
      for (int a = 0; a < alphabet; ++a) {
        double need = 0.5 * E(a, a);
        for (int b = 0; b < alphabet; ++b)
          if (b != a) need = fmax(need, E(a, b) - e[b]);
        if (need < e[a]) {
          e[a] = need;
          moved = true;
        }
      }
      if (!moved) break;
    }
    for (int a = 0; a < alphabet; ++a) e[a] += 9.094947017729282e-13;
  }
  double rmin = 0.0, rmax = 0.0;
  for (int a = 0; a < alphabet && a < 32; ++a) {
    double n = 0.0;
    for (int j = 0; j < 4; ++j) n += coords[a * 8 + j] * coords[a * 8 + j];
    T->r[a] = T->ok ? 0.5 * s * s * n - e[a] : 0.0;
    if (a == 0 || T->r[a] < rmin) rmin = T->r[a];
    if (a == 0 || T->r[a] > rmax) rmax = T->r[a];
  }
  const int32_t rmin64 = (int32_t)floor(rmin * 64.0), rmax64 = (int32_t)floor(rmax * 64.0);
  int32_t mid = rmin64 + (rmax64 - rmin64) / 2;
  if (mid > rmin64 + 2160) mid = rmin64 + 2160;
  T->rpos64 = mid;
  T->s2_half = 0.5 * s * s;
  for (int i = 0; i < 1024; ++i) {
    const uint64_t v = (uint64_t)T->bits[i & 31] | ((uint64_t)T->bits[i >> 5] << 24);
    T->pair[i].x = (uint32_t)v;
    T->pair[i].y = (uint32_t)(v >> 32);
  }
  if (e_out)
    for (int a = 0; a < 32; ++a) e_out[a] = e[a];
  if (s_out) *s_out = s;
}

__host__ __device__ inline void hs_j6_put(uint32_t (&w)[4], int bit, uint32_t c) {
  const int i = bit >> 5, sh = bit & 31;
  w[i] |= c << sh;
  if (sh > 26 && i < 3) w[i + 1] |= c >> (32 - sh);
}

__host__ __device__ inline void hs_j6_record(double rho, int k, int32_t rpos64, uint32_t pos24_bits,
                                             uint32_t (&rec)[4], int64_t* enc64) {
  const int64_t v64 = (int64_t)floor(rho * 64.0) - 1, rho0 = (int64_t)k * rpos64;
  const int64_t w = rho0 - v64;
  int64_t Q = w >= 0 ? w / 240 : -((-w + 239) / 240);
  int64_t rem = w - 240 * Q;
  if (Q < -HS_J6_QMAX) {
    Q = -HS_J6_QMAX;
    rem = 0;
  }
  if (Q > HS_J6_QMAX) {
    Q = HS_J6_QMAX;
    rem = 239;
  }
  if (enc64) *enc64 = rho0 - (240 * Q + rem);
  rec[0] = pos24_bits & 0xffffffu;
  rec[1] = rec[2] = rec[3] = 0u;
  for (int j = 0; j < HS_J6_NC; ++j) {
    const int take = (int)(Q > 15 ? 15 : Q < -15 ? -15 : Q);
    Q -= take;
    hs_j6_put(rec, 24 + 6 * j, hs_e2m3_code(4 * take));
  }
  hs_j6_put(rec, 24 + 6 * HS_J6_NC, hs_e2m3_code(4 * (int)(rem >> 4)));
  hs_j6_put(rec, 24 + 6 * (HS_J6_NC + 1), hs_e2m3_code((int)(rem & 15)));
}

__host__ __device__ inline void hs_j6_query_consts(uint32_t (&w)[6]) {
  for (int i = 0; i < 6; ++i) w[i] = 0u;
  for (int j = 0; j < HS_J6_NC + 2; ++j) {
    const uint32_t c = j < HS_J6_NC ? 31u : j == HS_J6_NC ? 4u : 1u;
    const int bit = 24 + 6 * j, i = bit >> 5, sh = bit & 31;
    w[i] |= c << sh;
    if (sh > 26) w[i + 1] |= c >> (32 - sh);
  }
}

#define HS_J6_CMAX (1 << 23)
__host__ __device__ inline int64_t hs_j6_query_c64(double sum_r, double s2_half, double r2, int k, int32_t rpos64) {
  const double g = sum_r - s2_half * r2;
  const int64_t g64 = (int64_t)floor(g * 64.0) - 1;
  return -(g64 + (int64_t)k * rpos64);
}
```

### hsearch_amd/csrc/hs_join8.hip

```cpp
#include <stdio.h>
#include <stdlib.h>
#include <string.h>

#include <algorithm>

#include "hs_internal.h"

namespace {

typedef int intx4 __attribute__((ext_vector_type(4)));
typedef int intx16 __attribute__((ext_vector_type(16)));

constexpr int QD = 4;
constexpr int HS_J8_CONST_AT = 48;
__host__ __device__ constexpr int ks_of(int k, bool wide = false) {
  return wide ? (k <= 20 ? 6 : 8) : k <= 25 ? 4 : k <= 41 ? 6 : 8;
}
constexpr uint32_t JRES = 256;
__device__ __forceinline__ void close_reservation(uint2* __restrict__ prov, uint32_t res_base, uint32_t res_used,
                                                  uint32_t prov_cap, int lane) {
  for (uint32_t i = res_used + (uint32_t)lane; i < JRES; i += 64u)
    if (res_base + i < prov_cap) prov[res_base + i] = make_uint2(0xffffffffu, 0u);
}
constexpr int DIG = 13;
// ... 1753 lines not shown
    if ((uint32_t)tid < kept) out[s_base + (uint32_t)tid] = s_keep[tid];
    __syncthreads();
    if (tid == 0) s_n = 0;
    __syncthreads();
  }
}

template <int PW>
__global__ __launch_bounds__(256) void hs_refine_codes_kernel(hs_tables_dev tabs,
                                                              const uint2* __restrict__ prov,
                                                              const uint32_t* __restrict__ prov_count,
                                                              uint32_t prov_cap,
                                                              const uint32_t* __restrict__ sorted_ql,
                                                              const uint4* __restrict__ qpacked,
                                                              const double* __restrict__ coords, int alphabet,
                                                              int k, int L, double r2_call,
                                                              const double* __restrict__ radii,
                                                              const uint32_t* __restrict__ qstart,
                                                              const uint32_t* __restrict__ qcount,
                                                              uint2* __restrict__ out,
                                                              uint32_t* __restrict__ out_count) {
  constexpr int NPOS = 25 * PW;
  constexpr int U = 4;
  __shared__ double s_x[32 * 8];
  __shared__ float s_T[32 * 32];
  __shared__ uint2 s_keep[256 * U];
  __shared__ uint32_t s_n, s_base;
  const int tid = threadIdx.x;
  s_x[tid] = tid < alphabet * 8 ? coords[tid] : 0.0;
  if (tid == 0) s_n = 0;
  __syncthreads();
  for (int e = tid; e < 32 * 32; e += 256) {
    const int x = e >> 5, c = e & 31;
    double t = 0.0;
#pragma unroll
    for (int j = 0; j < 8; ++j) {
      const double d = s_x[x * 8 + j] - s_x[c * 8 + j];
      t += d * d;
    }
    s_T[e] = (x < alphabet && c < alphabet) ? __double2float_rz(t) : 0.f;
  }
  __syncthreads();
  const uint32_t n = min(*prov_count, prov_cap);
  const float thr_call = hs_filter_bound(r2_call);
  for (uint32_t base = blockIdx.x * (256u * U); base < n; base += gridDim.x * (256u * U)) {
    uint32_t ql[U], pos[U], fs_id[U];
    bool live[U], pass[U];
    uint4 pk[U][PW], qk[U][PW];
#pragma unroll
    for (int u = 0; u < U; ++u) {
      const uint32_t e = base + (uint32_t)(u * 256 + tid);
      const uint2 raw = e < n ? prov[e] : make_uint2(0xffffffffu, 0u);
      ql[u] = raw.x;
      pos[u] = raw.y;
      live[u] = raw.x != 0xffffffffu;
    }
#pragma unroll
    for (int u = 0; u < U; ++u)
      if (live[u] && (ql[u] & HS_PROV_INDIRECT)) ql[u] = sorted_ql[ql[u] & ~HS_PROV_INDIRECT];
#pragma unroll
    for (int u = 0; u < U; ++u) {
      const uint32_t q = live[u] ? ql[u] / (uint32_t)L : 0u, l = live[u] ? ql[u] % (uint32_t)L : 0u;
#pragma unroll
      for (int w = 0; w < PW; ++w) {
        pk[u][w] = tabs.t[l].packed[(uint64_t)(live[u] ? pos[u] : 0u) * PW + w];
        qk[u][w] = qpacked[(uint64_t)q * PW + w];
      }
    }
#pragma unroll
    for (int u = 0; u < U; ++u) {
      const uint32_t q = live[u] ? ql[u] / (uint32_t)L : 0u, l = live[u] ? ql[u] % (uint32_t)L : 0u;
      const Stream256 sm = stitch<PW>(pk[u][0], pk[u][PW - 1]), sq = stitch<PW>(qk[u][0], qk[u][PW - 1]);
      const float thr = radii ? hs_filter_bound(hs_r2_of(radii, q, r2_call)) : thr_call;
      float s = 0.f;
#define HS_R(P) \
  if ((P) < NPOS && (P) < k) s += s_T[(stream_at<5 * (P)>(sm) << 5) | stream_at<5 * (P)>(sq)];
#define HS_R10(P) HS_R(P) HS_R(P + 1) HS_R(P + 2) HS_R(P + 3) HS_R(P + 4) HS_R(P + 5) HS_R(P + 6) HS_R(P + 7) HS_R(P + 8) HS_R(P + 9)
      HS_R10(0) HS_R10(10) HS_R(20) HS_R(21) HS_R(22) HS_R(23) HS_R(24)
      if constexpr (PW == 2) { HS_R10(25) HS_R10(35) HS_R(45) HS_R(46) HS_R(47) HS_R(48) HS_R(49) }
#undef HS_R10
#undef HS_R
      pass[u] = live[u] && !(s > thr);
      fs_id[u] = (pass[u] && l) ? tabs.t[l].ids[pos[u]] : 0u;
    }
#pragma unroll
    for (int u = 0; u < U; ++u) {
      const uint32_t q = live[u] ? ql[u] / (uint32_t)L : 0u;
      const int l = live[u] ? (int)(ql[u] % (uint32_t)L) : 0;
      if (__ballot(pass[u] && l > 0))
        pass[u] = pass[u] && !seen_in_earlier_table(tabs, qstart, qcount, q, l, L, fs_id[u], pass[u]);
    }
#pragma unroll
    for (int u = 0; u < U; ++u)
      if (pass[u]) s_keep[atomicAdd(&s_n, 1u)] = make_uint2(ql[u], pos[u]);
    __syncthreads();
    const uint32_t kept = s_n;
    if (tid == 0 && kept) s_base = atomicAdd(out_count, kept);
    __syncthreads();
    for (uint32_t i = (uint32_t)tid; i < kept; i += 256u) out[s_base + i] = s_keep[i];
    __syncthreads();
    if (tid == 0) s_n = 0;
    __syncthreads();
  }
}

inline unsigned blocks_for(uint64_t n, unsigned per = 256) { return (unsigned)((n + per - 1) / per); }

}

hipError_t hs_launch_jtables8(const double* d_coords, int alphabet, void* d_tab8, float* d_scale,
                              uint32_t* d_unsafe, void* d_tabR, void* d_tabW, hipStream_t s) {
  hs_jtables8_kernel<<<1, 32, 0, s>>>(d_coords, alphabet, (uint4*)d_tab8, d_scale, d_unsafe, (uint4*)d_tabR,
                                      (uint4*)d_tabW);
  return hipGetLastError();
}

hipError_t hs_launch_qprep8(const double* d_centers, uint32_t nq, int k, int wide, double r2,
                            const float* d_scale, void* d_c8, uint32_t* d_unsafe, void* d_c8b,
                            hipStream_t s, const double* d_radii) {
  if (!nq) return hipSuccess;
  if (wide)
    hs_qprep8_kernel<true><<<blocks_for(nq, 4), 256, 0, s>>>(d_centers, nq, k, r2, d_scale, (int8_t*)d_c8,
                                                             d_unsafe, nullptr, d_radii);
  else
    hs_qprep8_kernel<false><<<blocks_for(nq, 4), 256, 0, s>>>(d_centers, nq, k, r2, d_scale, (int8_t*)d_c8,
                                                              d_unsafe, (int8_t*)d_c8b, d_radii);
  return hipGetLastError();
}

hipError_t hs_launch_qprep8_codes(const uint8_t* d_qcodes, uint32_t nq, int k, int wide, double r2,
                                  const double* d_coords, const void* d_tab8, const void* d_tabR,
                                  const void* d_tabW, const float* d_scale, void* d_c8, void* d_c8b,
                                  hipStream_t s, const double* d_radii) {
  if (!nq) return hipSuccess;
  if (wide)
    hs_qprep8_codes_kernel<true><<<blocks_for(nq), 256, 0, s>>>(d_qcodes, nq, k, r2, d_coords, (const uint4*)d_tab8,
                                                                (const uint4*)d_tabR, (const uint4*)d_tabW,
                                                                d_scale, (int8_t*)d_c8, nullptr, d_radii);
  else
    hs_qprep8_codes_kernel<false><<<blocks_for(nq), 256, 0, s>>>(d_qcodes, nq, k, r2, d_coords, (const uint4*)d_tab8,
                                                                 (const uint4*)d_tabR, (const uint4*)d_tabW,
                                                                 d_scale, (int8_t*)d_c8, (int8_t*)d_c8b, d_radii);
  return hipGetLastError();
}

int hs_join8_row_bytes(int k, int wide) { return 32 * ks_of(k, wide != 0); }
uint32_t hs_join8_members_per_item(int k, int wide) {
  const int KS = ks_of(k, wide != 0);
  return (KS == 4 || (wide && KS == 6)) ? 128u : 64u;
}

hipError_t hs_launch_gather_c8t(const void* d_c8, const uint32_t* d_sorted_ql, const uint32_t* d_seg_qoff,
                                const uint32_t* d_seg_of, uint32_t nql, int L, int k, int wide, void* d_out,
                                hipStream_t s, int pieces) {
  if (!nql) return hipSuccess;
  hs_gather_c8t_kernel<<<blocks_for((uint64_t)nql * 8), 256, 0, s>>>((const int8_t*)d_c8, d_sorted_ql, d_seg_qoff, d_seg_of, nql,
                                                       L, pieces ? pieces : 2 * ks_of(k, wide != 0), (uint4*)d_out);
  return hipGetLastError();
}

uint32_t hs_join8_chunk_items(uint32_t n_items, int n_blocks, double pairs_per_item, uint32_t chunk) {
  const uint32_t n_waves = (uint32_t)n_blocks * 4u;
  uint32_t g_max = 8u;
  if (pairs_per_item > 0.0) g_max = (uint32_t)std::max(8.0, std::min(48.0, 7.0e5 / pairs_per_item));
  const uint32_t g_small = std::min(8u, n_items / (n_waves * 8u));
  return chunk ? chunk : std::max(2u, std::min(g_max, std::max(g_small, n_items / (n_waves * 64u))));
}

hipError_t hs_launch_join8w(const uint4* d_desc, uint32_t n_items, const uint4* d_packed_base,
                            const uint4* d_rec_base, const void* d_c8t, const void* d_tab8, int k, int wide,
                            uint32_t* d_prov_count, uint32_t prov_cap, uint2* d_prov,
                            uint32_t* d_item_counter, int n_blocks, const uint32_t* d_n_items,
                            double pairs_per_item, uint32_t xcd_run, hipStream_t s, uint32_t chunk) {
  if (!n_items) return hipSuccess;
  const uint32_t G = hs_join8_chunk_items(n_items, n_blocks, pairs_per_item, chunk);
#define HS_J8(JT_, KS_)                                                                               \
  hs_join8w_kernel<JT_, KS_><<<n_blocks, 256, 0, s>>>(d_desc, n_items, d_packed_base, d_rec_base,     \
                                                      (const uint4*)d_c8t, (const uint4*)d_tab8,      \
                                                      d_prov_count, prov_cap, d_prov, d_item_counter, G, \
                                                      d_n_items)
  const int KS = ks_of(k, wide != 0);
  if (wide && KS == 6)
    hs_join8xw_kernel<<<n_blocks, 256, 0, s>>>(d_desc, n_items, d_packed_base, d_rec_base, (const uint4*)d_c8t,
                                               (const uint4*)d_tab8, d_prov_count, prov_cap, d_prov, d_item_counter,
                                               G, d_n_items);
  else if (wide)
    hs_join8w_kernel<2, 8, true><<<n_blocks, 256, 0, s>>>(d_desc, n_items, d_packed_base, d_rec_base,
                                                          (const uint4*)d_c8t, (const uint4*)d_tab8, d_prov_count,
                                                          prov_cap, d_prov, d_item_counter, G, d_n_items);
  else if (KS == 4)
    hs_join8x_kernel<<<n_blocks, 256, 0, s>>>(d_desc, n_items, d_packed_base, d_rec_base, (const uint4*)d_c8t,
                                              (const uint4*)d_tab8, d_prov_count, prov_cap, d_prov,
                                              d_item_counter, G, d_n_items, xcd_run);
  else if (KS == 6) HS_J8(2, 6);
  else HS_J8(2, 8);
#undef HS_J8
#ifdef HS_JOIN_TIMING
  {
    unsigned long long t[8];
    (void)hipStreamSynchronize(s);
    (void)hipMemcpyFromSymbol(t, HIP_SYMBOL(g_join8_timing), sizeof(t));
    fprintf(stderr, "join8 timing (wave-cycles): chunk %llu build %llu next-desc+issue %llu first group %llu other groups %llu flush %llu member-wait %llu | longest wave %llu, mean wave %llu\n",
            t[0], t[1], t[2], t[3], t[4], t[5], t[6], t[7],
            (t[0] + t[1] + t[2] + t[3] + t[4] + t[5] + t[6]) / (unsigned long long)(n_blocks * 4));
    memset(t, 0, sizeof(t));
    (void)hipMemcpyToSymbol(HIP_SYMBOL(g_join8_timing), t, sizeof(t));
  }
#endif
  return hipGetLastError();
}

hipError_t hs_launch_join8r(const uint4* d_desc, uint32_t desc_cap, const uint32_t* d_split,
                            const uint4* d_packed_base, const uint32_t* d_rho_base, const void* d_c8t,
                            const void* d_tab8, int alphabet, uint32_t* d_prov_count, uint32_t prov_cap,
                            uint2* d_prov, uint32_t* d_item_counter, int n_blocks, double pairs_per_item,
                            hipStream_t s) {
  if (!desc_cap) return hipSuccess;
  if (alphabet < 1 || alphabet > HS_JR_MAX_ALPHABET) return hipErrorInvalidValue;
  const J8rLayout lay = join8r_layout(alphabet);
  {
    static int granted = 0;
    if ((int)lay.total > granted) {
      hipError_t e = hipFuncSetAttribute(reinterpret_cast<const void*>(hs_join8r_kernel),
                                         hipFuncAttributeMaxDynamicSharedMemorySize, (int)lay.total);
      if (e != hipSuccess) return e;
      granted = (int)lay.total;
    }
  }
  uint32_t G = 16u;
  if (pairs_per_item > 0.0) G = (uint32_t)std::max(8.0, std::min(64.0, 1.4e5 / pairs_per_item * 8.0));
  const uint32_t n_waves = (uint32_t)n_blocks * 4u;
  G = std::max(2u, std::min(G, std::max(2u, desc_cap / (n_waves * 32u))));
  hs_join8r_kernel<<<n_blocks, 256, lay.total, s>>>(d_desc, d_split, desc_cap, d_packed_base, d_rho_base,
                                                    (const uint4*)d_c8t, (const uint4*)d_tab8, alphabet, d_prov_count,
                                                    prov_cap, d_prov, d_item_counter, G);
  return hipGetLastError();
}

hipError_t hs_launch_gather_rec8(const uint4* d_packed_all, const uint32_t* d_ids_sorted, uint32_t n,
                                 int k, int wide, const void* d_tab8, const void* d_tabW, const float* d_scale,
                                 uint4* d_out_packed, uint4* d_out_rec, uint32_t* d_out_rho, hipStream_t s) {
  if (!n) return hipSuccess;
  hs_gather_rec8_kernel<<<blocks_for(n), 256, 0, s>>>(d_packed_all, d_ids_sorted, n, k, hs_packed_words(k), wide,
                                                      (const uint4*)d_tab8, (const uint4*)d_tabW, d_scale,
                                                      d_out_packed, d_out_rec, d_out_rho);
  return hipGetLastError();
}

hipError_t hs_launch_refine8(const hs_tables_dev& tabs, const uint2* d_prov, const uint32_t* d_prov_count,
                             uint32_t prov_cap, const uint32_t* d_sorted_ql, const void* d_c8,
                             const void* d_c8b, const void* d_tabR, const float* d_scale, int k, int L,
                             const uint32_t* d_qstart, const uint32_t* d_qcount,
                             uint2* d_out, uint32_t* d_out_count, hipStream_t s) {
  if (k <= 25)
    hs_refine8_kernel<1><<<1024, 256, 0, s>>>(tabs, d_prov, d_prov_count, prov_cap, d_sorted_ql,
                                              (const int8_t*)d_c8, (const int8_t*)d_c8b, (const uint4*)d_tabR,
                                              d_scale, k, L, d_qstart, d_qcount, d_out, d_out_count);
  else
    hs_refine8_kernel<2><<<1024, 256, 0, s>>>(tabs, d_prov, d_prov_count, prov_cap, d_sorted_ql,
                                              (const int8_t*)d_c8, (const int8_t*)d_c8b, (const uint4*)d_tabR,
                                              d_scale, k, L, d_qstart, d_qcount, d_out, d_out_count);
  return hipGetLastError();
}

hipError_t hs_launch_refine_codes(const hs_tables_dev& tabs, const uint2* d_prov, const uint32_t* d_prov_count,
                                  uint32_t prov_cap, const uint32_t* d_sorted_ql, const uint4* d_qpacked,
                                  const double* d_coords, int alphabet, int k, int L, double r2,
                                  const double* d_radii, const uint32_t* d_qstart, const uint32_t* d_qcount,
                                  uint2* d_out, uint32_t* d_out_count, hipStream_t s) {
  if (alphabet < 1 || alphabet > HS_ALPHABET_PAD || k < 1 || k > 50 || !d_qpacked) return hipErrorInvalidValue;
  if (k <= 25)
    hs_refine_codes_kernel<1><<<1024, 256, 0, s>>>(tabs, d_prov, d_prov_count, prov_cap, d_sorted_ql, d_qpacked,
                                                   d_coords, alphabet, k, L, r2, d_radii, d_qstart, d_qcount, d_out,
                                                   d_out_count);
  else
    hs_refine_codes_kernel<2><<<1024, 256, 0, s>>>(tabs, d_prov, d_prov_count, prov_cap, d_sorted_ql, d_qpacked,
                                                   d_coords, alphabet, k, L, r2, d_radii, d_qstart, d_qcount, d_out,
                                                   d_out_count);
  return hipGetLastError();
}
```

### include/hsearch.h

```cpp
#ifndef HSEARCH_H
#define HSEARCH_H

#include <stddef.h>
#include <stdint.h>

#ifdef __cplusplus
extern "C" {
#endif

#define HS_API __attribute__((visibility("default")))

typedef enum hs_status {
  HS_OK = 0,
  HS_ERR_INVALID = 1,
  HS_ERR_NO_DEVICE = 2,
  HS_ERR_HIP = 3,
  HS_ERR_CAPACITY = 4,
  HS_ERR_STATE = 5,
  HS_ERR_KEY_COLLISION = 6,
  HS_ERR_NOMEM = 7,
  HS_ERR_IO = 8,
  HS_ERR_PEER = 9
} hs_status;

typedef struct hs_params {
  uint32_t k;
  uint32_t K;
  uint32_t L;
  double W;
  int32_t device;
  uint32_t alphabet;
} hs_params;

typedef struct hs_handle hs_handle;

typedef struct hs_profile {
  double ms_hash;
  double ms_sort;
  double ms_gather;
  double ms_probe;
  double ms_verify;
  double ms_finalize;
  double ms_total;
  uint64_t candidates;
  uint64_t provisional;
  uint64_t hits;
  uint64_t verify_launches;
  uint64_t join_batches;
  double ms_join;
  uint64_t join_items;
  uint64_t join_pairs;
  uint64_t join_pairs_issued;
  uint64_t join_i8_batches;
  uint64_t hash_values;
  uint64_t hash_flagged;
  uint32_t join_row_bytes;
  uint32_t join_wide;
  uint64_t join_items_resident;
  uint64_t join_async_retries;
  uint64_t queries_recognised;
  uint64_t join_f6_batches;
  uint64_t append_rebuilds;
  uint64_t append_new_buckets;
} hs_profile;

typedef struct hs_index_info {
  uint64_t n;
  uint64_t device_bytes;
  uint64_t n_buckets[32];
  uint64_t max_bucket[32];
  uint32_t key_seed;
} hs_index_info;


HS_API hs_status hs_create(const hs_params* params, const double* a, const double* b,
                           const double* coords, hs_handle** out);
HS_API void hs_destroy(hs_handle* h);
HS_API hs_status hs_set_planes(hs_handle* h, const double* a, const double* b);
HS_API const char* hs_last_error(const hs_handle* h);
HS_API hs_status hs_get_profile(const hs_handle* h, hs_profile* out);
HS_API hs_status hs_get_params(const hs_handle* h, hs_params* out);
HS_API hs_status hs_set_verify_mode(hs_handle* h, int mode);
HS_API hs_status hs_set_hash_mode(hs_handle* h, int mode, double eps_scale);
typedef enum hs_option {
  HS_OPT_QUERY_BATCH = 1,
  HS_OPT_SEG_MODE = 2,
  HS_OPT_JOIN_RESIDENT = 3,
  HS_OPT_RECOGNISE_KMERS = 4,
  HS_OPT_BUILD_GROUPING = 5,
  HS_OPT_WIDE_ROWS = 6,
  HS_OPT_REFINE8 = 7,
  HS_OPT_SELF_CODES = 8,
  HS_OPT_SORT_HITS = 10,
  HS_OPT_SYNC_ITEMS = 11,
  HS_OPT_JOIN_MIN_Q = 12,
  HS_OPT_JOIN_MIN_M = 13,
  HS_OPT_SORT_FROM_BIT = 14,
  HS_OPT_BUILD_SERIAL = 15,
  HS_OPT_PROBE_RECORDS = 17,
  HS_OPT_JOIN_CHUNK = 18,
  HS_OPT_SUMMARY_CHUNK = 19,
  HS_OPT_SUMMARY_ROWS = 20,
  HS_OPT_MSF_EDGE_BUDGET = 21,
  HS_OPT_JOIN_F6 = 22,
  HS_OPT_JOIN_XCD_RUN = 16
} hs_option;
HS_API hs_status hs_set_option(hs_handle* h, int option, int64_t value);

HS_API hs_status hs_join6_tables(const double* coords, uint32_t alphabet, double* s, uint8_t* codes, double* e,
                                 double* r, uint32_t* pair);
HS_API hs_status hs_join6_thresholds(const double* coords, uint32_t alphabet, const uint8_t* kmers, uint64_t n,
                                     uint32_t k, const double* r2, int64_t* rho64, int64_t* c64, int64_t* rho0_64,
                                     uint32_t* rec);
HS_API hs_status hs_join6_selftest(int device, int variant, uint64_t* mismatches, uint32_t* first_bad);
HS_API hs_status hs_set_bucket_partition(hs_handle* h, uint32_t part, uint32_t n_parts);
HS_API hs_status hs_set_multiprobe(hs_handle* h, uint32_t extra_probes);
HS_API hs_status hs_probe_buckets(hs_handle* h, const double* centers, uint64_t nq, int32_t* buckets, uint8_t* valid);
HS_API hs_status hs_wait_event(hs_handle* h, void* hip_event);
HS_API const char* hs_version(void);


HS_API hs_status hs_embed_codes(hs_handle* h, const uint8_t* codes, uint64_t n, double* out);

HS_API hs_status hs_hash_codes(hs_handle* h, const uint8_t* codes, uint64_t n, int32_t* buckets);
HS_API hs_status hs_hash_points(hs_handle* h, const double* points, uint64_t n, int32_t* buckets);

HS_API uint32_t hs_key_string(const int32_t* buckets, uint32_t K, char* out, uint32_t cap);
HS_API uint64_t hs_key_fingerprint(const int32_t* buckets, uint32_t K, uint32_t seed);
HS_API int hs_key_strings_equal(const int32_t* x, const int32_t* y, uint32_t K);


HS_API hs_status hs_index_build(hs_handle* h, const uint8_t* codes, uint64_t n);

HS_API hs_status hs_index_build_subset(hs_handle* h, const uint8_t* codes_all, uint64_t n_all,
                                       const uint32_t* subset, uint64_t n_subset);

HS_API hs_status hs_index_build_windows(hs_handle* h, const uint8_t* residues, uint64_t n_residues,
                                        const uint64_t* seq_start, uint64_t n_seq,
                                        uint64_t* n_windows, uint32_t* window_pos);
HS_API hs_status hs_index_shard_begin(hs_handle* h, const uint8_t* codes, uint64_t n, uint32_t rank,
                                      uint32_t world, uint64_t* block_lo, uint64_t* block_count);
HS_API hs_status hs_index_shard_hash_dev(hs_handle* h, uint32_t l, uint32_t seed, uint64_t* d_fp_block);
HS_API hs_status hs_index_shard_group_dev(hs_handle* h, uint32_t l, const uint64_t* d_fp_all, uint32_t* n_buckets);
HS_API hs_status hs_index_shard_tuples_dev(hs_handle* h, uint32_t l, int32_t* d_tuples);
HS_API hs_status hs_index_shard_finish_dev(hs_handle* h, uint32_t l, const int32_t* d_tuples_all,
                                           uint32_t* collided);
HS_API hs_status hs_index_shard_end(hs_handle* h, uint32_t key_seed);

HS_API hs_status hs_index_save(hs_handle* h, const char* path);
HS_API hs_status hs_index_load(hs_handle* h, const char* path);
HS_API hs_status hs_index_file_check(const char* path, char* err, uint32_t err_cap);

HS_API hs_status hs_index_append(hs_handle* h, const uint8_t* codes, uint64_t m);
HS_API hs_status hs_index_append_dev(hs_handle* h, const uint8_t* d_codes, uint64_t m);
HS_API hs_status hs_index_append_windows(hs_handle* h, const uint8_t* residues, uint64_t n_residues,
                                         const uint64_t* seq_start, uint64_t n_seq,
                                         uint64_t* n_windows, uint32_t* window_pos);

HS_API hs_status hs_index_table_append(const uint32_t* ids, const uint64_t* dir_key, const uint32_t* dir_start,
                                       const int32_t* dir_tuple, uint64_t n, uint64_t nb,
                                       const int32_t* block_ints, uint64_t m, uint32_t K, uint32_t seed,
                                       uint32_t* out_ids, uint64_t* out_dir_key, uint32_t* out_dir_start,
                                       int32_t* out_dir_tuple, uint64_t dir_cap, uint64_t* nb_out, uint32_t* collided);

#define HS_KLSH_NONE 0xffffffffffffffffull
HS_API hs_status hs_klsh_draw_planes(uint32_t feat, uint32_t bits, double sigma, double* w, double* b,
                                     double* t);
HS_API hs_status hs_klsh_codes(int device, const uint8_t* classes, uint64_t n_residues,
                               const uint64_t* seq_start, uint64_t n_seq, const double* w,
                               const double* b, const double* t, uint32_t bits, uint64_t* codes,
                               uint64_t* uncertain, char* err, uint32_t err_cap);

HS_API hs_status hs_index_info_get(const hs_handle* h, hs_index_info* out);


HS_API hs_status hs_query(hs_handle* h, const double* centers, uint64_t nq, double R,
                          uint32_t* hit_q, uint32_t* hit_id, uint32_t* hit_table, double* hit_dist,
                          uint64_t cap, uint64_t* n_hits, uint64_t* cand);
HS_API hs_status hs_query_dev(hs_handle* h, const double* d_centers, uint64_t nq, double R,
                              uint32_t* d_hit_q, uint32_t* d_hit_id, uint32_t* d_hit_table,
                              double* d_hit_dist, uint64_t cap, uint64_t* n_hits,
                              uint64_t* d_cand);

HS_API hs_status hs_query_codes(hs_handle* h, const uint8_t* qcodes, uint64_t nq, double R,
                                uint32_t* hit_q, uint32_t* hit_id, uint32_t* hit_table, double* hit_dist,
                                uint64_t cap, uint64_t* n_hits, uint64_t* cand);
HS_API hs_status hs_query_codes_dev(hs_handle* h, const uint8_t* d_qcodes, uint64_t nq, double R,
                                    uint32_t* d_hit_q, uint32_t* d_hit_id, uint32_t* d_hit_table,
                                    double* d_hit_dist, uint64_t cap, uint64_t* n_hits,
                                    uint64_t* d_cand);

HS_API hs_status hs_merge_first_table_dev(hs_handle* h, uint32_t* d_q, uint32_t* d_id, uint32_t* d_table,
                                          double* d_dist, uint64_t n, uint64_t* n_out);


HS_API hs_status hs_query_radii(hs_handle* h, const double* centers, const uint8_t* qcodes, uint64_t nq,
                                const double* radii, uint32_t* hit_q, uint32_t* hit_id, uint32_t* hit_table,
                                double* hit_dist, uint64_t cap, uint64_t* n_hits, uint64_t* cand);
HS_API hs_status hs_query_radii_dev(hs_handle* h, const double* d_centers, const uint8_t* d_qcodes, uint64_t nq,
                                    const double* d_radii, uint32_t* d_hit_q, uint32_t* d_hit_id,
                                    uint32_t* d_hit_table, double* d_hit_dist, uint64_t cap, uint64_t* n_hits,
                                    uint64_t* d_cand);
HS_API hs_status hs_bruteforce_radii(hs_handle* h, const double* centers, uint64_t nq, const double* radii,
                                     uint32_t* hit_q, uint32_t* hit_id, double* hit_dist, uint64_t cap,
                                     uint64_t* n_hits);


HS_API hs_status hs_annotate(hs_handle* h, const double* centers, const uint8_t* qcodes, uint64_t nq, double R,
                             const double* radii, uint32_t* out_id, uint32_t* out_q, uint32_t* out_table,
                             double* out_dist, uint64_t cap, uint64_t* n_out);
HS_API hs_status hs_annotate_dev(hs_handle* h, const double* d_centers, const uint8_t* d_qcodes, uint64_t nq, double R,
                                 const double* d_radii, uint32_t* d_out_id, uint32_t* d_out_q, uint32_t* d_out_table,
                                 double* d_out_dist, uint64_t cap, uint64_t* n_out);
HS_API hs_status hs_merge_best(const uint32_t* id, const uint32_t* q, const uint32_t* table, const double* dist,
                               uint64_t n, uint32_t* out_id, uint32_t* out_q, uint32_t* out_table, double* out_dist,
                               uint64_t cap, uint64_t* n_out);


HS_API hs_status hs_bruteforce(hs_handle* h, const double* centers, uint64_t nq, double R,
                               uint32_t* hit_q, uint32_t* hit_id, double* hit_dist, uint64_t cap,
                               uint64_t* n_hits);
HS_API hs_status hs_bruteforce_topk(hs_handle* h, const double* centers, uint64_t nq,
                                    uint32_t topk, uint32_t* nn_id, double* nn_dist2);


HS_API hs_status hs_self_join(hs_handle* h, double R, int sqrt_test, uint32_t* edge_i,
                              uint32_t* edge_j, uint32_t* edge_table, double* edge_dist,
                              uint64_t cap, uint64_t* n_edges);

HS_API hs_status hs_self_join_range(hs_handle* h, uint64_t first, uint64_t count, double R,
                                    int sqrt_test, uint32_t* edge_i, uint32_t* edge_j,
                                    uint32_t* edge_table, double* edge_dist, uint64_t cap,
                                    uint64_t* n_edges);


HS_API hs_status hs_components(hs_handle* h, double R, int sqrt_test, uint32_t* label, uint64_t* n_components,
                               uint64_t* n_edges);
HS_API hs_status hs_components_range(hs_handle* h, uint64_t first, uint64_t count, double R, int sqrt_test,
                                     uint32_t* label, uint64_t* n_components, uint64_t* n_edges);
HS_API hs_status hs_components_dev(hs_handle* h, double R, int sqrt_test, uint32_t* d_label, uint64_t* n_components,
                                   uint64_t* n_edges);
HS_API hs_status hs_components_range_dev(hs_handle* h, uint64_t first, uint64_t count, double R, int sqrt_test,
                                         uint32_t* d_label, uint64_t* n_components, uint64_t* n_edges);
HS_API hs_status hs_components_merge(const uint32_t* labels, uint64_t m, uint64_t n, uint32_t* out_label,
                                     uint64_t* n_components);


#define HS_NOISE 0xffffffffu
typedef struct hs_dbscan_counts {
  uint64_t n_clusters, n_core, n_border, n_noise, n_edges;
} hs_dbscan_counts;
HS_API hs_status hs_degrees(hs_handle* h, double R, int sqrt_test, uint32_t* degree, uint64_t* n_edges);
HS_API hs_status hs_degrees_range(hs_handle* h, uint64_t first, uint64_t count, double R, int sqrt_test,
                                  uint32_t* degree, uint64_t* n_edges);
HS_API hs_status hs_dbscan(hs_handle* h, double R, int sqrt_test, uint32_t min_pts, uint32_t* label, uint32_t* degree,
                           hs_dbscan_counts* out);
HS_API hs_status hs_degrees_dev(hs_handle* h, double R, int sqrt_test, uint32_t* d_degree, uint64_t* n_edges);
HS_API hs_status hs_degrees_range_dev(hs_handle* h, uint64_t first, uint64_t count, double R, int sqrt_test,
                                      uint32_t* d_degree, uint64_t* n_edges);
HS_API hs_status hs_dbscan_dev(hs_handle* h, double R, int sqrt_test, uint32_t min_pts, uint32_t* d_label,
                               uint32_t* d_degree, hs_dbscan_counts* out);
HS_API hs_status hs_dbscan_edges(const uint32_t* ei, const uint32_t* ej, uint64_t n_edges, uint64_t n,
                                 uint32_t min_pts, uint32_t* label, uint32_t* degree, hs_dbscan_counts* out);


typedef struct hs_msf_info {
// ... 124 lines not shown
```

Baseline: 21.69 million.

## Repack join6 query tiles into 128-byte rows with swizzled full-tile layout

Query rows for the FP6 MFMA join are now 128 bytes (8 pieces) instead of 112. The per-row threshold is folded into the unused B operand lanes, and a dedicated gather kernel lays full 32-row tiles out so each lane does two contiguous 16-byte loads. The MFMA now accumulates from zero and the survivor test compares against -C in float, replacing the old sign and AND-tree trick. This aims to cut load instructions and address math in the hot join loop, at the cost of more memory per query row and an extra path for partial tiles.

```diff
diff --git a/hsearch_amd/capi.py b/hsearch_amd/capi.py
--- a/hsearch_amd/capi.py
+++ b/hsearch_amd/capi.py
@@ -30,7 +30,7 @@
            "hs_density_tree_cut", "hs_query_topk", "hs_query_topk_dev", "hs_self_knn", "hs_self_knn_range",
            "hs_self_knn_dev", "hs_self_knn_range_dev", "hs_topk_merge", "hs_seq_match", "hs_seq_match_dev",
            "hs_window_id_start", "hs_seq_match_hits", "hs_seq_match_merge", "hs_join6_tables", "hs_join6_thresholds",
-           "hs_join6_selftest", "hs_index_append", "hs_index_append_dev", "hs_index_append_windows",
+           "hs_join6_selftest", "hs_join6_tile_offset", "hs_index_append", "hs_index_append_dev", "hs_index_append_windows",
            "hs_index_table_append"]
 
 TOPK_MAX = 64
@@ -616,6 +616,12 @@
     return dict(rho64=rho64, c64=c64, rho0_64=rho0.value, rec=rec)
 
 
+def join6_tile_offset(nr, row, piece):
+    f = load().hs_join6_tile_offset
+    f.restype = C.c_uint32
+    return int(f(C.c_uint32(nr), C.c_uint32(row), C.c_uint32(piece)))
+
+
 def join6_selftest(device=0, variant=0):
     n = C.c_uint64(0)
     bad = (C.c_uint32 * 4)()
diff --git a/hsearch_amd/csrc/hs_capi.hip b/hsearch_amd/csrc/hs_capi.hip
--- a/hsearch_amd/csrc/hs_capi.hip
+++ b/hsearch_amd/csrc/hs_capi.hip
@@ -2472,6 +2472,8 @@
   const double* radii = nullptr;
 };
 
+static size_t qrow_room() { return std::max<size_t>(208 * 2, 128 + (size_t)hs_join6_row_bytes()); }
+
 static hipError_t launch_qrows(hs_handle* h, const BatchPlan& p, const Batch& b, hipStream_t s) {
   const int k = (int)h->p.k;
   uint32_t* const d_unsafe = h->counters.as<uint32_t>() + 8;
@@ -2494,9 +2496,9 @@
 
 static hipError_t gather_qrows(hs_handle* h, const BatchPlan& p, const Batch& b) {
   if (p.f6) {
-    hipError_t e = hs_launch_gather_c8t(h->c16.as<char>() + (size_t)b.nq * 128, h->sorted_ql.as<uint32_t>(),
+    hipError_t e = hs_launch_gather_c6t(h->c16.as<char>() + (size_t)b.nq * 128, h->sorted_ql.as<uint32_t>(),
                                         h->seg_qoff.as<uint32_t>(), h->seg_of.as<uint32_t>(), b.nqs, (int)h->p.L,
-                                        (int)h->p.k, 0, c6t_of(h, b), h->stream, hs_join6_row_pieces());
+                                        c6t_of(h, b), h->stream);
     if (e != hipSuccess || !p.use_r) return e;
   }
   if (p.use_i8)
@@ -2551,7 +2553,7 @@
     }
   }
   if (p.use_join) {
-    HS_HIP(h, h->c16.reserve((size_t)b.nq * 208 * 2));
+    HS_HIP(h, h->c16.reserve((size_t)b.nq * qrow_room()));
     if (p.refine && !b.qcodes) HS_HIP(h, h->c8b.reserve((size_t)b.nq * hs_join8_row_bytes(k, p.wide)));
     HS_HIP(h, hipEventRecord(h->evx[EV_FORK], h->stream));
     HS_HIP(h, hipStreamWaitEvent(h->stream2, h->evx[EV_FORK], 0));
@@ -2598,7 +2600,7 @@
 static hs_status group_segments(hs_handle* h, const BatchPlan& p, Batch& b) {
   if (!p.use_join) return HS_OK;
   const size_t n1 = (size_t)b.nql + 1;
-  HS_HIP(h, h->c16s.reserve(((size_t)b.nql + 64) * 208 * 2));
+  HS_HIP(h, h->c16s.reserve(((size_t)b.nql + 64) * qrow_room()));
   for (DevBuf* d : {&h->seg_keys, &h->seg_keys_sorted, &h->seg_key}) HS_HIP(h, d->reserve(n1 * 8));
   for (DevBuf* d : {&h->seg_vals, &h->sorted_ql, &h->seg_cnt, &h->seg_qoff, &h->seg_items, &h->item_off, &h->seg_of})
     HS_HIP(h, d->reserve(n1 * 4));
diff --git a/hsearch_amd/csrc/hs_internal.h b/hsearch_amd/csrc/hs_internal.h
--- a/hsearch_amd/csrc/hs_internal.h
+++ b/hsearch_amd/csrc/hs_internal.h
@@ -486,13 +486,15 @@
                                   uint2* d_out, uint32_t* d_out_count, hipStream_t s);
 hipError_t hs_launch_gather_c8t(const void* d_c8, const uint32_t* d_sorted_ql, const uint32_t* d_seg_qoff,
                                 const uint32_t* d_seg_of, uint32_t nql, int L, int k, int wide, void* d_out,
-                                hipStream_t s, int pieces = 0 );
+                                hipStream_t s);
 int hs_join8_row_bytes(int k, int wide);
 uint32_t hs_join8_members_per_item(int k, int wide);
 uint32_t hs_join8_chunk_items(uint32_t n_items, int n_blocks, double pairs_per_item, uint32_t chunk);
 size_t hs_join6_table_bytes();
 size_t hs_join6_ok_offset();
-int hs_join6_row_pieces();
+int hs_join6_row_bytes();
+hipError_t hs_launch_gather_c6t(const void* d_c6, const uint32_t* d_sorted_ql, const uint32_t* d_seg_qoff,
+                                const uint32_t* d_seg_of, uint32_t nql, int L, void* d_out, hipStream_t s);
 hipError_t hs_launch_jtables6(const double* d_coords, int alphabet, void* d_tab6, hipStream_t s);
 hipError_t hs_launch_gather_rec6(const uint4* d_packed_all, const uint32_t* d_ids_sorted, uint32_t n, int k,
                                  const void* d_tab6, uint4* d_out_rec, hipStream_t s);
diff --git a/hsearch_amd/csrc/hs_join6.hip b/hsearch_amd/csrc/hs_join6.hip
--- a/hsearch_amd/csrc/hs_join6.hip
+++ b/hsearch_amd/csrc/hs_join6.hip
@@ -11,12 +11,14 @@
 
 namespace {
 
+typedef int intx3 __attribute__((ext_vector_type(3)));
+typedef int intx4 __attribute__((ext_vector_type(4)));
 typedef int intx6 __attribute__((ext_vector_type(6)));
 typedef int intx8 __attribute__((ext_vector_type(8)));
 typedef float floatx4 __attribute__((ext_vector_type(4)));
 
 constexpr uint32_t JRES = 256;
-constexpr int PIECES = 7;
+constexpr int PIECES = HS_J6_ROW_BYTES / 16;
 
 __device__ __forceinline__ void close_reservation(uint2* __restrict__ prov, uint32_t res_base, uint32_t res_used,
                                                   uint32_t prov_cap, int lane) {
@@ -30,9 +32,8 @@
 }
 
 template <int SCALE = 0>
-__device__ __forceinline__ floatx4 tile_mfma6(const intx6 a, const intx6 b, const floatx4 c) {
+__device__ __forceinline__ floatx4 tile_mfma6(const intx6 a, const intx8 b8, const floatx4 c) {
   const intx8 a8 = __builtin_shufflevector(a, a, 0, 1, 2, 3, 4, 5, -1, -1);
-  const intx8 b8 = __builtin_shufflevector(b, b, 0, 1, 2, 3, 4, 5, -1, -1);
   return __builtin_amdgcn_mfma_scale_f32_16x16x128_f8f6f4(a8, b8, c, 2, 2, 0, SCALE, 0, SCALE);
 }
 
@@ -109,56 +110,72 @@
   int64_t c64 = hs_j6_query_c64(sum_r, T->s2_half, r2, k, T->rpos64);
   c64 = c64 > HS_J6_CMAX ? HS_J6_CMAX : c64 < -HS_J6_CMAX ? -HS_J6_CMAX : c64;
   if (!(r2 == r2)) c64 = -HS_J6_CMAX;
-  uint32_t* row = out + (uint64_t)q * (PIECES * 4);
+  const uint32_t cbits = __float_as_uint((float)c64 * (1.0f / 64.0f));
+  uint4* row = reinterpret_cast<uint4*>(out) + (uint64_t)q * PIECES;
 #pragma unroll
   for (int a = 0; a < 4; ++a) {
-#pragma unroll
-    for (int i = 0; i < 4; ++i) row[4 * a + i] = W[a][i];
-    row[16 + 4 * (a >> 1) + 2 * (a & 1)] = W[a][4];
-    row[16 + 4 * (a >> 1) + 2 * (a & 1) + 1] = W[a][5];
-  }
-  row[24] = __float_as_uint((float)c64 * (1.0f / 64.0f));
-  row[25] = row[26] = row[27] = 0u;
-}
-
-__device__ __forceinline__ void load_btile6(intx6 (&B)[2], float (&C)[2], const uint4* __restrict__ c6t,
-                                            uint32_t row0, uint32_t nr, int lane) {
-  const char* t0 = reinterpret_cast<const char*>(c6t + (uint64_t)row0 * PIECES);
-  const uint32_t n = (uint32_t)lane & 15u, q = (uint32_t)lane >> 4;
+    row[a] = make_uint4(W[a][0], W[a][1], W[a][2], W[a][3]);
+    row[4 + a] = make_uint4(W[a][4], W[a][5], cbits, cbits);
+  }
+}
+
+__global__ __launch_bounds__(256) void hs_gather_c6t_kernel(const uint4* __restrict__ c6,
+                                                            const uint32_t* __restrict__ sorted_ql,
+                                                            const uint32_t* __restrict__ seg_qoff,
+                                                            const uint32_t* __restrict__ seg_of, uint32_t nql, int L,
+                                                            char* __restrict__ out) {
+  const uint32_t t = blockIdx.x * 256 + threadIdx.x;
+  const uint32_t p = t >> 3, g = t & 7u;
+  if (p >= nql) return;
+  const uint32_t lo = seg_of[p];
+  const uint32_t qoff = seg_qoff[lo], nQ = seg_qoff[lo + 1] - qoff;
+  const uint32_t local = p - qoff, tile = local >> 5, j = local & 31u;
+  const uint32_t nr = min(32u, nQ - (tile << 5));
+  const uint32_t q = sorted_ql[p] / (uint32_t)L;
+  char* dst = out + (uint64_t)(qoff + (tile << 5)) * HS_J6_ROW_BYTES + hs_j6_tile_offset(nr, j, g);
+  *reinterpret_cast<uint4*>(dst) = c6[(uint64_t)q * PIECES + g];
+}
+
+__device__ __forceinline__ void load_btile6(intx8 (&B)[2], const char* __restrict__ c6t, uint32_t row0, uint32_t nr,
+                                            int lane) {
+  const char* t0 = c6t + (uint64_t)row0 * HS_J6_ROW_BYTES;
+  const char* base = t0 + 16 * lane;
 #pragma unroll
   for (int c = 0; c < 2; ++c) {
-    const uint32_t row = min(16u * (uint32_t)c + n, nr - 1u);
-    const uint4 hi = *reinterpret_cast<const uint4*>(t0 + (q * nr + row) * 16u);
-    const uint2 lo = *reinterpret_cast<const uint2*>(t0 + ((4u + (q >> 1)) * nr + row) * 16u + 8u * (q & 1u));
-    C[c] = *reinterpret_cast<const float*>(t0 + (6u * nr + row) * 16u);
-    B[c] = intx6{(int)hi.x, (int)hi.y, (int)hi.z, (int)hi.w, (int)lo.x, (int)lo.y};
-  }
-}
-
-__device__ __forceinline__ void sign_step6(int g, const floatx4 (&acc)[4][2], int (&w)[16]) {
-  auto v = [&](int i) { return __float_as_int(acc[i >> 3][(i >> 2) & 1][i & 3]); };
-  if (g < 10) w[g] = max(max(v(3 * g), v(3 * g + 1)), v(3 * g + 2));
-  else if (g < 13) w[g] = max(max(w[3 * (g - 10)], w[3 * (g - 10) + 1]), w[3 * (g - 10) + 2]);
-  else if (g == 13) w[13] = max(max(w[9], v(30)), v(31));
-  else if (g == 14) w[14] = max(max(w[10], w[11]), w[12]);
-  else w[15] = max(w[13], w[14]);
+    const intx4 hi = *reinterpret_cast<const intx4*>(base + 2048 * c);
+    const intx3 lo = *reinterpret_cast<const intx3*>(base + 2048 * c + 1024);
+    B[c] = intx8{hi.x, hi.y, hi.z, hi.w, lo.x, lo.y, lo.z, 0};
+  }
+  if (__builtin_expect(nr != 32u, 0)) {
+    const uint32_t n = (uint32_t)lane & 15u, q = (uint32_t)lane >> 4;
+#pragma unroll
+    for (int c = 0; c < 2; ++c) {
+      const uint32_t row = min(16u * (uint32_t)c + n, nr - 1u);
+      const intx4 hi = *reinterpret_cast<const intx4*>(t0 + hs_j6_tile_offset(nr, row, q));
+      const intx3 lo = *reinterpret_cast<const intx3*>(t0 + hs_j6_tile_offset(nr, row, 4u + q));
+      B[c] = intx8{hi.x, hi.y, hi.z, hi.w, lo.x, lo.y, lo.z, 0};
+    }
+  }
+}
+
+__device__ __forceinline__ float max3f(float a, float b, float c) { return __builtin_fmaxf(__builtin_fmaxf(a, b), c); }
+__device__ __forceinline__ void sign_step6(int g, const floatx4 (&acc)[4][2], float (&w)[16]) {
+  const int c = g >> 3, s = g & 7, o = 8 * c;
+  auto v = [&](int i) { return acc[i >> 2][c][i & 3]; };
+  if (s < 5) w[g] = max3f(v(3 * s), v(3 * s + 1), v(3 * s + 2));
+  else if (s == 5) w[g] = max3f(w[o], w[o + 1], w[o + 2]);
+  else if (s == 6) w[g] = max3f(w[o + 3], w[o + 4], v(15));
+  else w[g] = max3f(w[o + 5], w[o + 6], v(15));
   asm volatile("" : "+v"(w[g]));
 }
-
-__device__ __forceinline__ uint32_t and_tree6(const floatx4 (&acc)[4][2]) {
-  uint32_t a = 0xffffffffu;
-#pragma unroll
-  for (int t = 0; t < 4; ++t)
-#pragma unroll
-    for (int c = 0; c < 2; ++c)
-#pragma unroll
-      for (int i = 0; i < 4; ++i) a &= __float_as_uint(acc[t][c][i]);
-  return a;
+__device__ __forceinline__ bool group_pass6(const float (&w)[16], const float (&C)[2]) {
+  return (w[7] >= -C[0]) | (w[15] >= -C[1]);
 }
 
 __device__ __forceinline__ void emit_survivors6(const floatx4 (&acc)[4][2], int T0, uint32_t qc, uint32_t qoff,
                                                 uint32_t q_end, uint32_t wbase, uint32_t M, uint32_t mstart,
-                                                int lane, uint32_t& res_base, uint32_t& res_used,
+                                                const float (&C)[2], int lane, uint32_t& res_base,
+                                                uint32_t& res_used,
                                                 uint32_t* __restrict__ prov_count, uint32_t prov_cap,
                                                 uint2* __restrict__ prov) {
   const uint32_t n = (uint32_t)lane & 15u, q = (uint32_t)lane >> 4;
@@ -166,12 +183,11 @@
   for (int t = 0; t < 4; ++t)
 #pragma unroll
     for (int c = 0; c < 2; ++c) {
-      const uint32_t any = __float_as_uint(acc[t][c][0]) & __float_as_uint(acc[t][c][1]) &
-                           __float_as_uint(acc[t][c][2]) & __float_as_uint(acc[t][c][3]);
-      if (!__ballot((int)any >= 0)) continue;
+      const float thr = -C[c];
       uint32_t mask = 0;
 #pragma unroll
-      for (int i = 0; i < 4; ++i) mask |= (__float_as_int(acc[t][c][i]) >= 0 ? 1u : 0u) << i;
+      for (int i = 0; i < 4; ++i) mask |= (acc[t][c][i] >= thr ? 1u : 0u) << i;
+      if (!__ballot(mask != 0)) continue;
       const uint32_t col = qc + 16u * (uint32_t)c + n;
       if (!(col < q_end)) mask = 0u;
       const uint32_t ql = HS_PROV_INDIRECT | (qoff + col);
@@ -206,7 +222,7 @@
 
 __global__ __launch_bounds__(256, 2) void hs_join6x_kernel(
     const uint4* __restrict__ desc, uint32_t n_items, const uint4* __restrict__ packed_base,
-    const uint4* __restrict__ rec_base, const uint4* __restrict__ c6t, const hs_j6_dev* __restrict__ T,
+    const uint4* __restrict__ rec_base, const char* __restrict__ c6t, const hs_j6_dev* __restrict__ T,
     uint32_t* __restrict__ prov_count, uint32_t prov_cap, uint2* __restrict__ prov,
     uint32_t* __restrict__ item_counter, uint32_t G, const uint32_t* __restrict__ n_items_dev, uint32_t xcd_run) {
   if (n_items_dev) n_items = min(n_items, __builtin_amdgcn_readfirstlane(*n_items_dev));
@@ -266,8 +282,7 @@
   uint4 mk[RT];
   constexpr int NB = 3;
   constexpr uint32_t GQ = 32 * NB;
-  intx6 Bq[NB][2];
-  float Cq[NB][2];
+  intx8 Bq[NB][2];
 #define HS_LOAD_MEMBERS(D0)                                                              \
   {                                                                                      \
     const int64_t off_ = (int64_t)(((uint64_t)(D0).y << 32) | (uint64_t)(D0).x);         \
@@ -282,7 +297,7 @@
 #define HS_LOAD_GROUP(ROW, Q0, QEND)                                                             \
   _Pragma("unroll") for (int u = 0; u < NB; ++u) {                                               \
     const uint32_t qu_ = (Q0) + 32u * u < (QEND) ? (Q0) + 32u * u : (Q0);                        \
-    load_btile6(Bq[u], Cq[u], c6t, (ROW) + qu_, min(32u, (QEND) - qu_), lane);                   \
+    load_btile6(Bq[u], c6t, (ROW) + qu_, min(32u, (QEND) - qu_), lane);                          \
   }
   HS_LOAD_MEMBERS(d0)
   {
@@ -321,6 +336,7 @@
 #pragma unroll
       for (int c = 0; c < 2; ++c) accY[t][c] = __builtin_nondeterministic_value(accY[t][c]);
     bool y_live = false;
+    float Cy[2] = {0.0f, 0.0f};
     uint32_t prev_qc = q_begin;
     const uint32_t n_groups = HS_N_GROUPS(d1);
     uint32_t qc0 = HS_FIRST_Q(d1);
@@ -335,52 +351,53 @@
 #pragma unroll
       for (int u = 0; u < NB; ++u) {
         const uint32_t qc = qc0 + 32u * (uint32_t)u;
-        intx6 (&B)[2] = Bq[u];
+        intx8 (&B)[2] = Bq[u];
         if (u == 0 || qc < q_end) {
-          const floatx4 Cv[2] = {floatx4{Cq[u][0], Cq[u][0], Cq[u][0], Cq[u][0]},
-                                 floatx4{Cq[u][1], Cq[u][1], Cq[u][1], Cq[u][1]}};
-          int wY[16];
+          const floatx4 zero = floatx4{0.0f, 0.0f, 0.0f, 0.0f};
+          const float Cx[2] = {__int_as_float(B[0][6]), __int_as_float(B[1][6])};
+          float wY[16];
 #pragma unroll
           for (int g = 0; g < 8; ++g) {
             const int t = g >> 1, c = g & 1;
-            accX[t][c] = tile_mfma6(A[t], B[c], Cv[c]);
+            accX[t][c] = tile_mfma6(A[t], B[c], zero);
             if (y_live) {
               sign_step6(2 * g, accY, wY);
               sign_step6(2 * g + 1, accY, wY);
             }
             __builtin_amdgcn_sched_barrier(0);
           }
-          const uint32_t sY = y_live ? (uint32_t)wY[15] : 0x80000000u;
-          if (y_live && __ballot((int)sY >= 0))
-            emit_survivors6(accY, 4, prev_qc, qoff, q_end, wbase, M, mstart, lane, res_base, res_used, prov_count,
-                            prov_cap, prov);
+          if (y_live && __ballot(group_pass6(wY, Cy)))
+            emit_survivors6(accY, 4, prev_qc, qoff, q_end, wbase, M, mstart, Cy, lane, res_base, res_used,
+                            prov_count, prov_cap, prov);
           y_live = true;
-          int wX[16];
+          float wX[16];
 #pragma unroll
           for (int g = 0; g < 8; ++g) {
             const int t = g >> 1, c = g & 1;
-            accY[t][c] = tile_mfma6(A[4 + t], B[c], Cv[c]);
+            accY[t][c] = tile_mfma6(A[4 + t], B[c], zero);
             sign_step6(2 * g, accX, wX);
             sign_step6(2 * g + 1, accX, wX);
             __builtin_amdgcn_sched_barrier(0);
           }
-          const uint32_t sX = (uint32_t)wX[15];
-          if (__ballot((int)sX >= 0))
-            emit_survivors6(accX, 0, qc, qoff, q_end, wbase, M, mstart, lane, res_base, res_used, prov_count,
+          if (__ballot(group_pass6(wX, Cx)))
+            emit_survivors6(accX, 0, qc, qoff, q_end, wbase, M, mstart, Cx, lane, res_base, res_used, prov_count,
                             prov_cap, prov);
           prev_qc = qc;
+          asm volatile("v_mov_b32 %0, %2\n\tv_mov_b32 %1, %3" : "=&v"(Cy[0]), "=v"(Cy[1]) : "v"(Cx[0]), "v"(Cx[1]));
         }
         const uint32_t nb = nq0 + 32u * (uint32_t)u < nqend ? nq0 + 32u * (uint32_t)u : nq0;
-        load_btile6(B, Cq[u], c6t, nrow + nb, min(32u, nqend - nb), lane);
+        load_btile6(B, c6t, nrow + nb, min(32u, nqend - nb), lane);
       }
       qc0 = nq0;
     };
     do_group(0);
     for (uint32_t gi = 1; gi < n_groups; ++gi) do_group(gi);
     {
-      const uint32_t sY = and_tree6(accY);
-      if (__ballot((int)sY >= 0))
-        emit_survivors6(accY, 4, prev_qc, qoff, q_end, wbase, M, mstart, lane, res_base, res_used, prov_count,
+      float wY[16];
+#pragma unroll
+      for (int g = 0; g < 16; ++g) sign_step6(g, accY, wY);
+      if (__ballot(group_pass6(wY, Cy)))
+        emit_survivors6(accY, 4, prev_qc, qoff, q_end, wbase, M, mstart, Cy, lane, res_base, res_used, prov_count,
                         prov_cap, prov);
     }
     if (!has_next) break;
@@ -443,7 +460,8 @@
   }
   const float cf = (float)st_c64(cs, n) * (1.0f / 64.0f);
   const floatx4 d = tile_mfma6<SCALE>(intx6{(int)a[0], (int)a[1], (int)a[2], (int)a[3], (int)a[4], (int)a[5]},
-                                      intx6{(int)b[0], (int)b[1], (int)b[2], (int)b[3], (int)b[4], (int)b[5]},
+                                      intx8{(int)b[0], (int)b[1], (int)b[2], (int)b[3], (int)b[4], (int)b[5],
+                                            __float_as_int(cf), __float_as_int(cf)},
                                       floatx4{cf, cf, cf, cf});
 #pragma unroll
   for (int i = 0; i < 4; ++i) {
@@ -474,7 +492,15 @@
 
 size_t hs_join6_table_bytes() { return sizeof(hs_j6_dev); }
 size_t hs_join6_ok_offset() { return offsetof(hs_j6_dev, ok); }
-int hs_join6_row_pieces() { return PIECES; }
+int hs_join6_row_bytes() { return HS_J6_ROW_BYTES; }
+
+hipError_t hs_launch_gather_c6t(const void* d_c6, const uint32_t* d_sorted_ql, const uint32_t* d_seg_qoff,
+                                const uint32_t* d_seg_of, uint32_t nql, int L, void* d_out, hipStream_t s) {
+  if (!nql) return hipSuccess;
+  hs_gather_c6t_kernel<<<blocks_for((uint64_t)nql * PIECES), 256, 0, s>>>((const uint4*)d_c6, d_sorted_ql, d_seg_qoff,
+                                                                          d_seg_of, nql, L, (char*)d_out);
+  return hipGetLastError();
+}
 
 hipError_t hs_launch_gather_rec6(const uint4* d_packed_all, const uint32_t* d_ids_sorted, uint32_t n, int k,
                                  const void* d_tab6, uint4* d_out_rec, hipStream_t s) {
@@ -497,7 +523,7 @@
                             uint32_t prov_cap, uint2* d_prov, uint32_t* d_item_counter, int n_blocks,
                             const uint32_t* d_n_items, uint32_t G, uint32_t xcd_run, hipStream_t s) {
   if (!n_items) return hipSuccess;
-  hs_join6x_kernel<<<n_blocks, 256, 0, s>>>(d_desc, n_items, d_packed_base, d_rec_base, (const uint4*)d_c6t,
+  hs_join6x_kernel<<<n_blocks, 256, 0, s>>>(d_desc, n_items, d_packed_base, d_rec_base, (const char*)d_c6t,
                                             (const hs_j6_dev*)d_tab6, d_prov_count, prov_cap, d_prov, d_item_counter,
                                             G, d_n_items, xcd_run);
   return hipGetLastError();
@@ -553,6 +579,11 @@
   return HS_OK;
 }
 
+HS_API uint32_t hs_join6_tile_offset(uint32_t nr, uint32_t row, uint32_t piece) {
+  if (nr < 1 || nr > 32 || row >= nr || piece >= (uint32_t)PIECES) return 0xffffffffu;
+  return hs_j6_tile_offset(nr, row, piece);
+}
+
 HS_API hs_status hs_join6_selftest(int device, int variant, uint64_t* mismatches, uint32_t* first_bad) {
   if (!mismatches || variant < 0 || variant > 1) return HS_ERR_INVALID;
   if (hipSetDevice(device) != hipSuccess) return HS_ERR_HIP;
diff --git a/hsearch_amd/csrc/hs_join6_tables.h b/hsearch_amd/csrc/hs_join6_tables.h
--- a/hsearch_amd/csrc/hs_join6_tables.h
+++ b/hsearch_amd/csrc/hs_join6_tables.h
@@ -160,3 +160,9 @@
   const int64_t g64 = (int64_t)floor(g * 64.0) - 1;
   return -(g64 + (int64_t)k * rpos64);
 }
+
+#define HS_J6_ROW_BYTES 128
+__host__ __device__ inline uint32_t hs_j6_tile_offset(uint32_t nr, uint32_t j, uint32_t g) {
+  if (nr == 32u) return ((2u * (j >> 4) + (g >> 2)) << 10) + 16u * (16u * (g & 3u) + (j & 15u));
+  return 16u * (g * nr + j);
+}
diff --git a/hsearch_amd/csrc/hs_join8.hip b/hsearch_amd/csrc/hs_join8.hip
--- a/hsearch_amd/csrc/hs_join8.hip
+++ b/hsearch_amd/csrc/hs_join8.hip
@@ -1929,10 +1929,10 @@
 
 hipError_t hs_launch_gather_c8t(const void* d_c8, const uint32_t* d_sorted_ql, const uint32_t* d_seg_qoff,
                                 const uint32_t* d_seg_of, uint32_t nql, int L, int k, int wide, void* d_out,
-                                hipStream_t s, int pieces) {
+                                hipStream_t s) {
   if (!nql) return hipSuccess;
   hs_gather_c8t_kernel<<<blocks_for((uint64_t)nql * 8), 256, 0, s>>>((const int8_t*)d_c8, d_sorted_ql, d_seg_qoff, d_seg_of, nql,
-                                                       L, pieces ? pieces : 2 * ks_of(k, wide != 0), (uint4*)d_out);
+                                                       L, 2 * ks_of(k, wide != 0), (uint4*)d_out);
   return hipGetLastError();
 }
 
diff --git a/include/hsearch.h b/include/hsearch.h
--- a/include/hsearch.h
+++ b/include/hsearch.h
@@ -112,6 +112,7 @@
 HS_API hs_status hs_join6_thresholds(const double* coords, uint32_t alphabet, const uint8_t* kmers, uint64_t n,
                                      uint32_t k, const double* r2, int64_t* rho64, int64_t* c64, int64_t* rho0_64,
                                      uint32_t* rec);
+HS_API uint32_t hs_join6_tile_offset(uint32_t nr, uint32_t row, uint32_t piece);
 HS_API hs_status hs_join6_selftest(int device, int variant, uint64_t* mismatches, uint32_t* first_bad);
 HS_API hs_status hs_set_bucket_partition(hs_handle* h, uint32_t part, uint32_t n_parts);
 HS_API hs_status hs_set_multiprobe(hs_handle* h, uint32_t extra_probes);
```

Result: faster. 23.15 million, median of 6 (+6.7%).
